# NJU-RLC/quadrupedal-agility

Hardware: AMD Instinct MI355X
Metric: env-steps/sec (4096 Go2 envs) + wall-clock to 1k PPO iters, 1/2/4/8 GPU (higher is better)
Workload: dtype f32

## Files before the change

### __graft_entry__.py

```python
import os
import shutil
import subprocess
import sys

ROOT = os.path.dirname(os.path.abspath(__file__))
CSRC = os.path.join(ROOT, "quadrupedal_agility_amd", "csrc")
if ROOT not in sys.path:
    sys.path.insert(0, ROOT)


def _hipcc():
    for cand in (shutil.which("hipcc"), "/opt/rocm/bin/hipcc"):
        if cand and os.path.exists(cand):
            return cand
    raise RuntimeError("hipcc not found")


def _src_hash(srcs):
    import hashlib
    h = hashlib.sha256()
    for s in srcs:
        h.update(os.path.basename(s).encode()); h.update(open(s, "rb").read())
    return h.hexdigest()


def _stale(out, srcs):
    stamp = out + ".srchash"
    if not os.path.exists(out) or not os.path.exists(stamp):
        return True
    return open(stamp).read().strip() != _src_hash(srcs)


HIP_SOURCES = (("qa_sim.hip", ["-fno-slp-vectorize", "-fno-hip-fp32-correctly-rounded-divide-sqrt"]), ("qa_learner.hip", []), ("qa_gemm.hip", []), ("qa_conv.hip", []),
               ("qa_policy.hip", []), ("qa_tsc.hip", ["-ffp-contract=off"]), ("qa_depth.hip", []))
HIP_HEADERS = ("qa_physics.h", "qa_device.h", "qa_go2_model.h", "qa_rewards.h")


def _lib_sources():
    srcs = [os.path.join(CSRC, f) for f, _ in HIP_SOURCES] + [os.path.join(CSRC, f) for f in HIP_HEADERS]
    srcs.append(os.path.join(ROOT, "include", "qa_sim.h"))
    srcs.append(os.path.join(ROOT, "include", "qa_sim_curriculum.h"))
    srcs.append(os.path.join(ROOT, "include", "qa_tsc_curriculum.h"))
    srcs.append(os.path.join(ROOT, "include", "qa_sim_rewards.h"))
    return srcs


def compile_library(out, obj_dir=None):
    base = [_hipcc(), "--offload-arch=gfx950", "-O3", "-std=c++17", "-fPIC"]
    obj_dir = obj_dir or os.path.dirname(out)
    objs = []
    for src, extra in HIP_SOURCES:
        obj = os.path.join(obj_dir, src.replace(".hip", ".o"))
        subprocess.check_call(base + extra + ["-c", os.path.join(CSRC, src), "-o", obj])
        objs.append(obj)
    subprocess.check_call([_hipcc(), "--offload-arch=gfx950", "-shared", "-fPIC", "-o", out] + objs)
    for obj in objs:
        os.remove(obj)


def build():
    srcs = _lib_sources()
    out = os.path.join(CSRC, "libqa_sim.so")
    if os.environ.get("QA_FORCE_REBUILD") == "1" or _stale(out, srcs):
        compile_library(out)
        with open(out + ".srchash", "w") as f:
            f.write(_src_hash(srcs))
    subprocess.check_call(["make", "-C", os.path.join(ROOT, "oracle"), "-s"])
    import quadrupedal_agility_amd
    from quadrupedal_agility_amd import _capi
    lib = _capi.load_library()
    assert lib.qa_abi_version() == _capi.QA_ABI_VERSION


def smoke():
    import numpy as np
    import torch
    from tests.oracle_lib import OracleSim, go2_cfg
    from quadrupedal_agility_amd.sim import QaSim
    assert torch.cuda.is_available(), "smoke() needs a GPU"
    n = 64
    q = go2_cfg(n, seed=1)
    o = OracleSim(q)
    h = QaSim(q, "cuda:0")
    o.reset_all()
    rng = np.random.default_rng(0)
    for _ in range(3):
        h.arena.copy_(torch.from_numpy(o.arena.copy()).cuda()); h.global_step = o.global_step
        act = rng.normal(0, 1, (n, 12)).astype(np.float32)
        o.step(act); h.step(torch.from_numpy(act).cuda())
        torch.cuda.synchronize()
        from tests.parity_tol import MEDIAN_TOL, env_mismatch, env_errors
        bad = np.zeros(n, bool)
        for name in ("OBS", "REW", "ROOT_STATES", "DOF_STATE", "OBS_DISC"):
            got, exp = h.t[name].cpu().numpy(), o.t[name]
            bad |= env_mismatch(name, got, exp, n)
            med = float(np.median(env_errors(name, got, exp, n)))
# ... 64 lines not shown
```

### quadrupedal_agility_amd/_capi.py

```python
import ctypes as C
import os

import torch

QA_ABI_VERSION = 18
NUM_DOF = 12
NUM_GAITS = 5
NUM_PROP = 57
HISTORY_LEN = 10
NUM_OBS = 671
NUM_OBS_DISC = 49
ACTION_BUF_LEN = 8
NUM_REWARDS = 14
MOCAP_FRAME = 37
MAX_MOCAP_CLIPS, MOCAP_CLIP = 64, 8
OBST_SEESAW, OBST_BAR, OBST_TYRE = 1, 2, 3

REWARD_NAMES = [
    "action_rate", "collision", "delta_torques", "dof_acc", "dof_error", "dof_pos_limits",
    "dof_vel_limits", "hip_pos", "jump_up_height", "locomotion_height", "torque_limits",
    "torques", "tracking_ang_vel", "tracking_lin_vel",
]

EXTRA_REWARD_NAMES = [
# ... 160 lines not shown
    f = getattr(lib, prefix + "tsc_goal_step"); f.argtypes = [C.c_void_p, C.c_void_p, C.c_void_p]; f.restype = C.c_int
    f = getattr(lib, prefix + "tsc_observations"); f.argtypes = [C.c_void_p, C.c_void_p, C.c_void_p]; f.restype = C.c_int
    f = getattr(lib, prefix + "tsc_depth_update"); f.argtypes = [C.c_void_p, C.c_void_p, C.c_void_p]; f.restype = C.c_int
    f = getattr(lib, prefix + "mlp_packed_floats"); f.argtypes = [C.c_void_p, C.c_int32]; f.restype = C.c_int64
    f = getattr(lib, prefix + "mlp_pack"); f.argtypes = [C.c_void_p, C.c_int32, C.c_void_p, C.c_void_p, C.c_void_p, C.c_int64, C.c_void_p]; f.restype = C.c_int
    f = getattr(lib, prefix + "mlp_strands"); f.argtypes = [C.c_void_p, C.c_int32, C.c_int32, C.c_void_p]; f.restype = C.c_int
    f = getattr(lib, prefix + "mlp_groups"); f.argtypes = [C.c_void_p, C.c_int32, C.c_int32, C.c_void_p, C.c_void_p, C.c_void_p, C.c_void_p]; f.restype = C.c_int
    f = getattr(lib, prefix + "mlp_set_groups"); f.argtypes = [C.c_int32]; f.restype = C.c_int
    f = getattr(lib, prefix + "mlp_forward")
    f.argtypes = [C.c_void_p, C.c_int64, C.c_int32, C.c_int32, C.c_void_p, C.c_int32, C.c_void_p, C.c_void_p, C.c_void_p, C.c_int32, C.c_void_p]
    f.restype = C.c_int
    f = getattr(lib, prefix + "elu_backward_bias")
    f.argtypes = [C.c_void_p] * 4 + [C.c_int64, C.c_int32, C.c_float, C.c_void_p, C.c_int64, C.c_void_p]
    f.restype = C.c_int
    f = getattr(lib, prefix + "narrow_wgrad_scratch_bytes"); f.argtypes = [C.c_int64, C.c_int32, C.c_int32]; f.restype = C.c_int64
    f = getattr(lib, prefix + "linear_forward")
    f.argtypes = [C.c_void_p, C.c_int64, C.c_void_p, C.c_int64, C.c_void_p, C.c_void_p, C.c_int64, C.c_int64, C.c_int32, C.c_int32, C.c_int32, C.c_float, C.c_void_p]
    f.restype = C.c_int
    f = getattr(lib, prefix + "linear_backward_input")
    f.argtypes = [C.c_void_p, C.c_int64, C.c_void_p, C.c_int64, C.c_void_p, C.c_int64, C.c_void_p, C.c_int64, C.c_int64, C.c_int32, C.c_int32, C.c_int32, C.c_float, C.c_void_p]
    f.restype = C.c_int
    f = getattr(lib, prefix + "linear_backward_weight_scratch_bytes"); f.argtypes = [C.c_int64, C.c_int32, C.c_int32]; f.restype = C.c_int64
    f = getattr(lib, prefix + "linear_backward_weight_layout"); f.argtypes = [C.c_int64, C.c_int32, C.c_int32, C.c_void_p]; f.restype = C.c_int
    f = getattr(lib, prefix + "linear_backward_weight_batch_layout"); f.argtypes = [C.c_int64, C.c_int32, C.c_int32, C.c_void_p]; f.restype = C.c_int
    f = getattr(lib, prefix + "linear_backward_weight_batch_scratch_bytes"); f.argtypes = [C.c_int64, C.c_int32, C.c_int32]; f.restype = C.c_int64
    f = getattr(lib, prefix + "linear_backward_weight_batch"); f.argtypes = [C.c_void_p, C.c_int32, C.c_void_p]; f.restype = C.c_int
    f = getattr(lib, prefix + "linear_backward_weight")
    f.argtypes = [C.c_void_p, C.c_int64, C.c_void_p, C.c_int64, C.c_void_p, C.c_void_p, C.c_int64, C.c_int32, C.c_int32, C.c_void_p, C.c_int64, C.c_void_p]
    f.restype = C.c_int
    f = getattr(lib, prefix + "tsc_reset_stats"); f.argtypes = [C.c_void_p, C.c_void_p, C.c_int64, C.c_int32, C.c_float, C.c_void_p, C.c_void_p, C.c_void_p]; f.restype = C.c_int
    f = getattr(lib, prefix + "slab_sum"); f.argtypes = [C.c_void_p, C.c_int64, C.c_int32, C.c_int64, C.c_void_p, C.c_void_p]; f.restype = C.c_int
    P, I64, I32, FL = C.c_void_p, C.c_int64, C.c_int32, C.c_float
    f = getattr(lib, prefix + "linear_forward_split_scratch_bytes"); f.argtypes = [I64, I32, I32]; f.restype = C.c_int64
    f = getattr(lib, prefix + "linear_forward_split"); f.argtypes = [P, I64, P, I64, P, P, I64, I64, I32, I32, I32, FL, P, I64, P]; f.restype = C.c_int
    f = getattr(lib, prefix + "disc_sample_prepare"); f.argtypes = [C.POINTER(QaDiscSampleIo), I32, I32, P, P, P, P, P, FL, FL, P, P]; f.restype = C.c_int
    f = getattr(lib, prefix + "disc_step_tail_scratch_bytes"); f.argtypes = []; f.restype = C.c_int64
    f = getattr(lib, prefix + "disc_step_tail"); f.argtypes = [P, P, I64, I32, P, P, I32, P, P, P, P, I32, FL, P, I64, P]; f.restype = C.c_int
    f = getattr(lib, prefix + "depth_stem_forward"); f.argtypes = [P, P, P, P, P, I64, I32, I32, FL, P]; f.restype = C.c_int
    f = getattr(lib, prefix + "depth_stem_backward_scratch_bytes"); f.argtypes = []; f.restype = C.c_int64
    f = getattr(lib, prefix + "depth_stem_backward"); f.argtypes = [P, P, P, P, I64, I32, I32, P, I64, P]; f.restype = C.c_int
    f = getattr(lib, prefix + "conv_nhwc_forward"); f.argtypes = [P, P, P, P, I64, I32, I32, I32, I32, I32, I32, I32, FL, P]; f.restype = C.c_int
    f = getattr(lib, prefix + "conv_nhwc_backward_input"); f.argtypes = [P, P, P, P, I64, I32, I32, I32, I32, I32, I32, I32, FL, P]; f.restype = C.c_int
    f = getattr(lib, prefix + "conv_nhwc_backward_weight_scratch_bytes"); f.argtypes = [I64, I32, I32, I32, I32, I32, I32]; f.restype = C.c_int64
    f = getattr(lib, prefix + "conv_nhwc_backward_weight"); f.argtypes = [P, P, P, P, I64, I32, I32, I32, I32, I32, I32, P, I64, P]; f.restype = C.c_int
    f = getattr(lib, prefix + "elu_backward_pad"); f.argtypes = [P, P, P, P, I64, I32, I32, I32, I32, I32, FL, P]; f.restype = C.c_int
    f = getattr(lib, prefix + "narrow_wgrad"); f.argtypes = [C.c_void_p, C.c_void_p, C.c_int64, C.c_int32, C.c_int32, C.c_void_p, C.c_void_p, C.c_void_p, C.c_int64, C.c_void_p]; f.restype = C.c_int
    return lib


def bind_extensions(lib, prefix="qa_"):
    f = getattr(lib, prefix + "set_terrain_curriculum"); f.argtypes = [C.c_void_p] * 4 + [C.c_int32, C.c_int32, C.c_float, C.c_float]; f.restype = C.c_int
    f = getattr(lib, prefix + "tsc_obstacle_curriculum"); f.argtypes = [C.POINTER(QaTscObstCurr), C.c_void_p]; f.restype = C.c_int
    f = getattr(lib, prefix + "set_extra_rewards"); f.argtypes = [C.c_void_p, C.POINTER(QaExtraRewards)]; f.restype = C.c_int
    return lib


class QaExtraRewards(C.Structure):
    _fields_ = [("scale_dt", C.c_float * 10), ("base_height_target", C.c_float), ("max_contact_force", C.c_float), ("step_dt", C.c_float),
                ("num_scan_points", C.c_int32), ("scan_offsets", C.c_void_p), ("extra_episode_sums", C.c_void_p), ("feet_air_time", C.c_void_p),
                ("extra_episode_stats", C.c_void_p)]


class QaTscObstCurr(C.Structure):
    _fields_ = [("step_counter", C.c_void_p), ("counter_offset", C.c_void_p), ("success_rate", C.c_void_p), ("any_reset", C.c_void_p),
                ("threshold", C.c_double), ("period", C.c_int64), ("state", C.c_void_p), ("ticket", C.c_void_p), ("increments", C.c_void_p),
                ("biases", C.c_void_p), ("last", C.c_int32), ("reserved", C.c_int32),
                ("cell_index", C.c_void_p), ("cell_kind", C.c_void_p), ("cell_base", C.c_void_p), ("num_cells", C.c_int64),
                ("height_samples", C.c_void_p), ("scan_samples", C.c_void_p), ("map_cells", C.c_int64),
                ("ceiling_index", C.c_void_p), ("ceiling_base", C.c_void_p), ("num_ceiling_cells", C.c_int64), ("ceiling_samples", C.c_void_p),
                ("goal_index", C.c_void_p), ("goal_kind", C.c_void_p), ("goal_base", C.c_void_p), ("num_goal_entries", C.c_int64),
                ("env_goals", C.c_void_p), ("goal_floats", C.c_int64)]


TSC_OBST_BAR, TSC_OBST_TYRE, TSC_OBST_STATE_WORDS = 0, 1, 4


class QaMlpOp(C.Structure):
    _fields_ = [("kind", C.c_int32), ("src_buf", C.c_int32), ("src_col", C.c_int32), ("dst_buf", C.c_int32), ("dst_col", C.c_int32),
                ("k", C.c_int32), ("n", C.c_int32), ("act", C.c_int32), ("out_index", C.c_int32), ("flags", C.c_int32),
                ("w_off", C.c_int64), ("b_off", C.c_int64), ("out_col", C.c_int32), ("aux_index", C.c_int32), ("aux_col", C.c_int32), ("pad_", C.c_int32)]


class QaWgradDesc(C.Structure):
    _fields_ = [("grad_out", C.c_void_p), ("ldg", C.c_int64), ("x", C.c_void_p), ("ldx", C.c_int64), ("grad_weight", C.c_void_p), ("grad_bias", C.c_void_p),
                ("rows", C.c_int64), ("in_features", C.c_int32), ("out_features", C.c_int32), ("scratch", C.c_void_p), ("scratch_bytes", C.c_int64)]


ADAM_STACK_MAX_TENSORS, ADAM_STACK_MAX_STATES = 16, 3


class QaPairJob(C.Structure):
    _fields_ = [("a", C.c_void_p), ("b", C.c_void_p), ("rows", C.c_int64), ("cols", C.c_int32), ("mode", C.c_int32), ("b_stride", C.c_int64),
                ("grad_scale", C.c_void_p), ("grad_a", C.c_void_p), ("out", C.c_void_p)]


class QaAdamPair(C.Structure):
    _fields_ = [("split_tensor", C.c_int32), ("split_chunk", C.c_int32), ("lr2", C.c_void_p), ("max_norm2", C.c_float), ("kl", C.c_void_p),
                ("desired_kl", C.c_float), ("kl_factor", C.c_float), ("lr_min", C.c_float), ("lr_max", C.c_float)]


class QaAdamStackState(C.Structure):
    _fields_ = [("exp_avg", C.c_void_p), ("exp_avg_sq", C.c_void_p), ("step", C.c_void_p), ("lr", C.c_void_p), ("weight_decay", C.c_float), ("pad_", C.c_int32)]


class QaAdamStackTensor(C.Structure):
    _fields_ = [("param", C.c_void_p), ("grad", C.c_void_p), ("tmp", C.c_void_p), ("src1", C.c_void_p), ("src2", C.c_void_p), ("stride1", C.c_int64), ("stride2", C.c_int64),
                ("parts1", C.c_int32), ("parts2", C.c_int32), ("alpha2", C.c_float), ("reg", C.c_float), ("numel", C.c_int32), ("num_states", C.c_int32),
# ... 24 lines not shown


TSC_GOAL_IO_FIELDS = ("root_states", "contact_forces", "rigid_body_states", "env_goals", "obstacle_types", "action_hl_history", "x_edge_mask",
                      "episode_length", "cur_goal_idx", "reach_goal_timer", "last_contacts", "cur_goals", "next_goals", "episode_sums",
                      "base_lin_vel", "base_ang_vel", "projected_gravity", "rpy", "contact_filt", "target_pos_rel", "next_target_pos_rel",
                      "target_yaw", "next_target_yaw", "reached_goal", "cur_obstacle_type", "reset_buf", "time_out_buf", "reach_goal_cutoff",
                      "rew_buf")


class QaTscGoalIo(C.Structure):
    _fields_ = [(name, C.c_void_p) for name in TSC_GOAL_IO_FIELDS]


class QaTscObsCfg(C.Structure):
    _fields_ = [("num_envs", C.c_int64), ("num_bodies", C.c_int32), ("key_bodies", C.c_int32 * 4), ("map_rows", C.c_int32), ("map_cols", C.c_int32),
                ("update_yaw", C.c_int32), ("root_height_obs", C.c_int32), ("action_stride", C.c_int64),
                ("points_env_stride", C.c_int64), ("point_stride", C.c_int32), ("reserved", C.c_int32),
                ("border_size", C.c_float), ("horizontal_scale", C.c_float), ("vertical_scale", C.c_float),
                ("lin_vel", C.c_float), ("ang_vel", C.c_float), ("dof_pos", C.c_float), ("dof_vel", C.c_float), ("lin_vel_dist", C.c_float),
                ("ang_vel_dist", C.c_float), ("key_pos", C.c_float), ("foot_contact", C.c_float), ("clip_observations", C.c_float),
                ("default_dof_pos", C.c_float * 12), ("default_dof_pos_all", C.c_float * 12)]


TSC_OBS_IO_FIELDS = ("root_states", "rpy", "base_lin_vel", "base_ang_vel", "contact_filt", "dof_pos", "dof_vel", "last_action",
                     "rigid_body_states", "mass_params", "friction", "motor_strength", "cur_obstacle_type", "target_yaw", "next_target_yaw",
                     "height_samples", "height_points", "commands", "latent_eps", "latent_c", "episode_length", "delta_yaw", "delta_next_yaw",
                     "obs_history", "measured_heights", "obs_buf", "obs_bbc_buf", "obs_disc_buf")
TSC_NUM_SCAN, TSC_NUM_OBS, TSC_NUM_OBS_BBC, TSC_NUM_OBS_DISC = 132, 800, 671, 49


class QaTscObsIo(C.Structure):
    _fields_ = [(name, C.c_void_p) for name in TSC_OBS_IO_FIELDS]


class QaTscDepthCfg(C.Structure):
    _fields_ = [("num_envs", C.c_int64), ("step", C.c_int64), ("seed", C.c_uint64), ("env_id_offset", C.c_int32), ("width", C.c_int32),
                ("height", C.c_int32), ("crop_top", C.c_int32), ("crop_bottom", C.c_int32), ("crop_left", C.c_int32), ("crop_right", C.c_int32),
                ("buffer_len", C.c_int32), ("map_rows", C.c_int32), ("map_cols", C.c_int32), ("coarse_log2", C.c_int32),
                ("horizontal_fov_deg", C.c_float), ("position", C.c_float * 3), ("near_clip", C.c_float), ("far_clip", C.c_float),
                ("depth_noise", C.c_float), ("border_size", C.c_float), ("horizontal_scale", C.c_float), ("vertical_scale", C.c_float)]


TSC_DEPTH_IO_FIELDS = ("root_states", "camera_pitch", "height_samples", "ceiling_samples", "episode_length", "depth_buffer", "coarse_floor_max",
                       "coarse_ceiling_min", "step_dev")


class QaTscDepthIo(C.Structure):
    _fields_ = [(name, C.c_void_p) for name in TSC_DEPTH_IO_FIELDS]


ABI_SYMBOLS = ["arena_bytes", "create", "destroy", "tensor_info", "env_step", "env_step_dev", "reset_all", "simulate",
               "set_mocap", "debug_post_physics", "env_physics_step", "tsc_reset", "tsc_reset_dev", "simulate_if", "gae", "ppo_loss", "ppo_loss_scratch_bytes", "hybrid_ppo_loss", "hybrid_ppo_loss_scratch_bytes", "elu_backward_bias",
               "elu_backward_bias_scratch_bytes", "narrow_wgrad", "narrow_wgrad_scratch_bytes", "linear_forward", "linear_backward_input", "linear_backward_weight", "linear_backward_weight_scratch_bytes", "linear_backward_weight_layout", "linear_backward_weight_batch", "linear_backward_weight_batch_layout", "linear_backward_weight_batch_scratch_bytes", "slab_sum", "linear_forward_split", "linear_forward_split_scratch_bytes", "depth_stem_forward", "depth_stem_backward", "depth_stem_backward_scratch_bytes", "conv_nhwc_forward", "conv_nhwc_backward_input", "conv_nhwc_backward_weight", "conv_nhwc_backward_weight_scratch_bytes", "elu_backward_pad", "normalizer_update", "normalizer_apply", "clip_adam_step", "clip_adam_step_hostgrads", "clip_adam_step_reduce", "clip_adam_pair_step", "grad_reduce", "adam_stack_step", "rollout_act", "rollout_act_store", "rollout_act_hybrid", "rollout_post", "rollout_post_amp", "disc_loss", "disc_loss_logits", "disc_loss_scratch_bytes", "disc_prepare", "disc_sample_prepare", "disc_step_tail", "disc_step_tail_scratch_bytes", "pair_loss", "pair_loss_scratch_bytes", "pair_losses", "pair_losses_scratch_bytes", "accumulate_scalars", "gather_rows", "kl_lr_rule", "episode_means", "set_lean_exports", "mlp_packed_floats", "mlp_pack", "mlp_forward", "mlp_strands", "mlp_groups", "mlp_set_groups", "tsc_set_commands", "tsc_goal_step", "tsc_observations", "tsc_depth_update", "tsc_reset_stats", "tsc_push", "tsc_start_pose", "tsc_reset_where", "last_error", "abi_version"]
EXTENSION_SYMBOLS = ["set_terrain_curriculum", "tsc_obstacle_curriculum", "set_extra_rewards"]

_LIB = None
LIB_PATH = os.environ.get("QA_LIB") or os.path.join(os.path.dirname(os.path.abspath(__file__)), "csrc", "libqa_sim.so")


def load_library():
    global _LIB
    if _LIB is None:
        if not os.path.exists(LIB_PATH):
            raise RuntimeError(
                f"{LIB_PATH} is missing: build it with `python -c 'import __graft_entry__ as g; g.build()'` "
                "(hipcc --offload-arch=gfx950). quadrupedal_agility_amd has no CPU fallback.")
        lib = C.CDLL(LIB_PATH)
        bind(lib, "qa_")
        bind_extensions(lib, "qa_")
        lib.qa_last_error.restype = C.c_char_p
        lib.qa_abi_version.restype = C.c_int
        if lib.qa_abi_version() != QA_ABI_VERSION:
            raise RuntimeError("libqa_sim.so ABI version mismatch")
        _LIB = lib
    return _LIB


def tensor_info(lib, prefix, cfg, which):
    off = C.c_int64(); shape = (C.c_int64 * 3)(); nd = C.c_int32(); dt = C.c_int32()
    rc = getattr(lib, prefix + "tensor_info")(C.byref(cfg), which, C.byref(off), shape, C.byref(nd), C.byref(dt))
    if rc != 0:
        raise RuntimeError(f"{prefix}tensor_info({which}) -> {rc}")
    return off.value, tuple(shape[i] for i in range(nd.value)), dt.value


def _ptr(t):
    return C.c_void_p(t.data_ptr())


def stream(on):
    dev = on if type(on) is torch.device else on.device
    return C.c_void_p(torch.cuda.current_stream(dev).cuda_stream) if dev.type == "cuda" else None


NO_ERROR_TEXT = "(an injected library: no error text)"


class Api:

    stream = staticmethod(stream)

    def __init__(self, lib=None, prefix="qa_"):
        self._lib, self.prefix = lib, prefix
        self._fns = {}

    @property
    def lib(self):
# ... 41 lines not shown
```

### quadrupedal_agility_amd/csrc/qa_learner.hip

```cpp
#include <hip/hip_runtime.h>
#include <stdint.h>
#include <stdio.h>

#include "../../include/qa_sim.h"
#include "../../include/qa_tsc_curriculum.h"
#include "qa_device.h"

namespace {

constexpr int PPO_BLOCK = 64;
constexpr int PPO_D = 12;
constexpr int PPO_SUMS = 5 + PPO_D;

struct PpoArgs {
    const float *mu, *std, *value, *actions, *old_logp, *old_mu, *old_sigma, *adv, *returns, *target_values;
    float *dmu, *dvalue;
    float *partial;
    int64_t B;
    float clip, c_surr, c_value, c_bound, c_entropy;
    int clipped_value;
};

__device__ __forceinline__ float wave_sum(float v) {
#pragma unroll
    for (int o = 32; o > 0; o >>= 1) v += __shfl_xor(v, o, 64);
    return v;
}

__global__ void __launch_bounds__(PPO_BLOCK) qa_ppo_loss_kernel(PpoArgs a) {
    const int64_t i = (int64_t)blockIdx.x * PPO_BLOCK + threadIdx.x;
    const bool live = i < a.B;
    const int64_t r = live ? i : a.B - 1;
    const float invB = 1.0f / (float)a.B;
    float sd[PPO_D];
#pragma unroll
    for (int j = 0; j < PPO_D; ++j) sd[j] = a.std[j];
    float mu[PPO_D], ac[PPO_D], omu[PPO_D], osd[PPO_D];
    {
        const float4 *m4 = (const float4 *)(a.mu + r * PPO_D), *a4 = (const float4 *)(a.actions + r * PPO_D);
        const float4 *om4 = (const float4 *)(a.old_mu + r * PPO_D), *os4 = (const float4 *)(a.old_sigma + r * PPO_D);
#pragma unroll
        for (int q = 0; q < 3; ++q) {
            float4 m = m4[q], x = a4[q], om = om4[q], os = os4[q];
            mu[4 * q] = m.x; mu[4 * q + 1] = m.y; mu[4 * q + 2] = m.z; mu[4 * q + 3] = m.w;
            ac[4 * q] = x.x; ac[4 * q + 1] = x.y; ac[4 * q + 2] = x.z; ac[4 * q + 3] = x.w;
            omu[4 * q] = om.x; omu[4 * q + 1] = om.y; omu[4 * q + 2] = om.z; omu[4 * q + 3] = om.w;
            osd[4 * q] = os.x; osd[4 * q + 1] = os.y; osd[4 * q + 2] = os.z; osd[4 * q + 3] = os.w;
        }
    }
    const float v = a.value[r], adv = a.adv[r], ret = a.returns[r], tv = a.target_values[r], ologp = a.old_logp[r];

    const float HALF_LOG_2PI = 0.91893853320467274178f;
    float logp = 0.f, ent = 0.f, kl = 0.f, bl = 0.f;
    float dlogp_dmu[PPO_D], dlogp_dsd[PPO_D], dbl_dmu[PPO_D];
#pragma unroll
    for (int j = 0; j < PPO_D; ++j) {
        const float s = sd[j], inv_s = 1.0f / s, d = ac[j] - mu[j], var = s * s, ls = logf(s);
        logp += -(d * d) / (2.0f * var) - ls - HALF_LOG_2PI;
        ent += 0.5f + HALF_LOG_2PI + ls;
        const float dm = omu[j] - mu[j];
        kl += logf(s / osd[j] + 1.0e-5f) + (osd[j] * osd[j] + dm * dm) / (2.0f * var) - 0.5f;
        dlogp_dmu[j] = d / var;
        dlogp_dsd[j] = d * d * inv_s * inv_s * inv_s - inv_s;
        const float lo = fminf(mu[j] + 1.0f, 0.0f), hi = fmaxf(mu[j] - 1.0f, 0.0f);
        bl += lo * lo + hi * hi;
        dbl_dmu[j] = 2.0f * lo + 2.0f * hi;
    }
    const float ratio = expf(logp - ologp);
    const float rc = fminf(fmaxf(ratio, 1.0f - a.clip), 1.0f + a.clip);
    const float s1 = -adv * ratio, s2 = -adv * rc;
    const float surr = fmaxf(s1, s2);
    const bool inside = ratio >= 1.0f - a.clip && ratio <= 1.0f + a.clip;
    float dsurr_dratio = s1 > s2 ? -adv : (s1 == s2 ? (inside ? -adv : -0.5f * adv) : 0.0f);
    const float dsurr_dlogp = dsurr_dratio * ratio;
    float vl, dvl_dv;
    if (a.clipped_value) {
        const float dv = v - tv, dvc = fminf(fmaxf(dv, -a.clip), a.clip), vc = tv + dvc;
        const float l1 = (v - ret) * (v - ret), l2 = (vc - ret) * (vc - ret);
        const float pass = (dv >= -a.clip && dv <= a.clip) ? 1.0f : 0.0f;
        vl = fmaxf(l1, l2);
        dvl_dv = l1 > l2 ? 2.0f * (v - ret) : (l1 == l2 ? (v - ret) + (vc - ret) * pass : 2.0f * (vc - ret) * pass);
    } else {
        vl = (ret - v) * (ret - v);
        dvl_dv = 2.0f * (v - ret);
    }
    if (live) {
        float g[PPO_D];
#pragma unroll
        for (int j = 0; j < PPO_D; ++j) g[j] = invB * (a.c_surr * dsurr_dlogp * dlogp_dmu[j] + a.c_bound * dbl_dmu[j]);
        float4 *o4 = (float4 *)(a.dmu + r * PPO_D);
        o4[0] = make_float4(g[0], g[1], g[2], g[3]); o4[1] = make_float4(g[4], g[5], g[6], g[7]); o4[2] = make_float4(g[8], g[9], g[10], g[11]);
        a.dvalue[r] = invB * a.c_value * dvl_dv;
    }
    const float w = live ? 1.0f : 0.0f;
    float part[PPO_SUMS];
    part[0] = w * surr; part[1] = w * vl; part[2] = w * bl; part[3] = w * ent; part[4] = w * kl;
#pragma unroll
    for (int j = 0; j < PPO_D; ++j) part[5 + j] = w * (a.c_surr * dsurr_dlogp * dlogp_dsd[j] - a.c_entropy / sd[j]);
#pragma unroll
    for (int k = 0; k < PPO_SUMS; ++k) {
        float s = wave_sum(part[k]);
        if (threadIdx.x == k) a.partial[(int64_t)blockIdx.x * PPO_SUMS + k] = s;
    }
}

__global__ void __launch_bounds__(256) qa_ppo_finish_kernel(const float *partial, int nblocks, int64_t B, float c_surr, float c_value,
                                                            float c_bound, float c_entropy, float *out, float *dstd) {
    constexpr int LANES = 256 / PPO_SUMS;
    __shared__ double s_acc[256];
    __shared__ double s_tot[PPO_SUMS];
    const int t = threadIdx.x;
    const int k = t / LANES, l = t % LANES;
    double acc = 0.0;
    if (k < PPO_SUMS)
        for (int b = l; b < nblocks; b += LANES) acc += (double)partial[(int64_t)b * PPO_SUMS + k];
    s_acc[t] = acc;
    __syncthreads();
    if (k < PPO_SUMS && l == 0) {
        double tot = 0.0;
        for (int q = 0; q < LANES; ++q) tot += s_acc[k * LANES + q];
        s_tot[k] = tot;
    }
    __syncthreads();
    const double invB = 1.0 / (double)B;
    if (t < 5) out[1 + t] = (float)(s_tot[t] * invB);
    if (t == 5) out[0] = (float)((c_surr * s_tot[0] + c_value * s_tot[1] + c_bound * s_tot[2] - c_entropy * s_tot[3]) * invB);
    if (t == 6 || t == 7) out[t] = 0.f;
    if (t >= 8 && t < 8 + PPO_D) dstd[t - 8] = (float)(s_tot[5 + t - 8] * invB);
}

constexpr int HYB_ND = 3, HYB_NC = 18, HYB_SUMS = 5 + HYB_NC;
struct HybArgs {
    const float *logits, *mean, *std, *value, *actions, *old_logp_d, *old_logp_c, *old_mu, *old_sigma, *adv, *returns, *target_values;
    float *dlogits, *dmean, *dvalue, *partial;
    int64_t B;
    float clip, c_value, c_entropy;
    int clipped_value;
};
__device__ __forceinline__ void clipped_surrogate(float logp, float ologp, float adv, float clip, float &surr, float &dsurr_dlogp) {
    const float ratio = expf(logp - ologp), rc = fminf(fmaxf(ratio, 1.0f - clip), 1.0f + clip);
    const float s1 = -adv * ratio, s2 = -adv * rc;
    surr = fmaxf(s1, s2);
    const bool inside = ratio >= 1.0f - clip && ratio <= 1.0f + clip;
    const float d = s1 > s2 ? -adv : (s1 == s2 ? (inside ? -adv : -0.5f * adv) : 0.0f);
    dsurr_dlogp = d * ratio;
}
__global__ void __launch_bounds__(PPO_BLOCK) qa_hybrid_ppo_loss_kernel(HybArgs a) {
    const int64_t i = (int64_t)blockIdx.x * PPO_BLOCK + threadIdx.x;
    const bool live = i < a.B;
    const int64_t r = live ? i : a.B - 1;
    const float invB = 1.0f / (float)a.B;
    const float HALF_LOG_2PI = 0.91893853320467274178f, EPS = 1.1920928955078125e-07f;
    float z[HYB_ND], pr[HYB_ND], lp[HYB_ND], fl[HYB_ND];
    float zmax = -3.0e38f;
#pragma unroll
    for (int k = 0; k < HYB_ND; ++k) { z[k] = a.logits[r * HYB_ND + k]; zmax = fmaxf(zmax, z[k]); }
    float den = 0.f;
#pragma unroll
    for (int k = 0; k < HYB_ND; ++k) { pr[k] = expf(z[k] - zmax); den += pr[k]; }
    float Hd = 0.f, sum_pf = 0.f;
#pragma unroll
    for (int k = 0; k < HYB_ND; ++k) {
        pr[k] /= den;
        fl[k] = (pr[k] > EPS && pr[k] < 1.0f - EPS) ? 1.0f : 0.0f;
        lp[k] = logf(fminf(fmaxf(pr[k], EPS), 1.0f - EPS));
        Hd -= pr[k] * lp[k];
        sum_pf += pr[k] * fl[k];
    }
    const float *act = a.actions + r * (1 + HYB_NC);
    int ad = (int)act[0];
    ad = ad < 0 ? 0 : (ad >= HYB_ND ? HYB_ND - 1 : ad);
    const float lpa = ad == 0 ? lp[0] : (ad == 1 ? lp[1] : lp[2]);
    const float fa = ad == 0 ? fl[0] : (ad == 1 ? fl[1] : fl[2]);
    const float adv = a.adv[r];
    float surr_d, dsd_dlogp;
    clipped_surrogate(lpa, a.old_logp_d[r], adv, a.clip, surr_d, dsd_dlogp);
    float logp = 0.f, ent_c = 0.f, kl = 0.f;
    float dlogp_dmu[HYB_NC], dlogp_dsd[HYB_NC], inv_sd[HYB_NC];
#pragma unroll
    for (int j = 0; j < HYB_NC; ++j) {
        const float s = a.std[j], inv_s = 1.0f / s, mu = a.mean[r * HYB_NC + j], d = act[1 + j] - mu, var = s * s, ls = logf(s);
// ... 295 lines not shown
    int num_chunks, num_tensors;
    float beta1, beta2, eps, max_norm;
    int inline_grads;
    const float *gin[QA_ADAM_MAX_INLINE];
    int has_reduce;
    const float *red_src[QA_ADAM_MAX_INLINE];
    int64_t red_stride[QA_ADAM_MAX_INLINE];
    int32_t red_parts[QA_ADAM_MAX_INLINE];
    int split_chunk, split_tensor;
    float *lr2; float max_norm2;
    const float *kl; float desired_kl, kl_factor, lr_min, lr_max;
};
__device__ __forceinline__ const float *adam_grad(const AdamArgs &a, int t) { return a.inline_grads ? a.gin[t] : a.grads[t]; }

constexpr int QA_REDUCE_WIDE = 16;
__device__ __forceinline__ float adam_reduce_chunk(const float *__restrict__ src, int64_t stride, int parts, float *__restrict__ g, int n, float *s_q) {
    float acc = 0.f;
    if (parts <= QA_REDUCE_WIDE) {
        for (int i = threadIdx.x; i < n; i += 256) {
            float v[QA_REDUCE_WIDE];
#pragma unroll
            for (int z = 0; z < QA_REDUCE_WIDE; ++z) v[z] = z < parts ? src[(int64_t)z * stride + i] : 0.f;
            float s = v[0];
#pragma unroll
            for (int z = 1; z < QA_REDUCE_WIDE; ++z) if (z < parts) s += v[z];
            g[i] = s;
            acc = fmaf(s, s, acc);
        }
    } else {
        const int c = threadIdx.x & 31, q = threadIdx.x >> 5;
        float a0 = 0.f, a1 = 0.f, a2 = 0.f, a3 = 0.f;
        if (c < n) {
            int b = q;
            for (; b + 24 < parts; b += 32) {
                a0 += src[(int64_t)b * stride + c]; a1 += src[(int64_t)(b + 8) * stride + c];
                a2 += src[(int64_t)(b + 16) * stride + c]; a3 += src[(int64_t)(b + 24) * stride + c];
            }
            for (; b < parts; b += 8) a0 += src[(int64_t)b * stride + c];
        }
        s_q[threadIdx.x] = (a0 + a1) + (a2 + a3);
        __syncthreads();
        if (q == 0 && c < n) {
            float t = 0.f;
#pragma unroll
            for (int k = 0; k < 8; ++k) t += s_q[threadIdx.x + 32 * k];
            g[c] = t;
            acc = t * t;
        }
        __syncthreads();
    }
    return acc;
}

__global__ void __launch_bounds__(256) qa_adam_sumsq_kernel(AdamArgs a) {
    __shared__ float s_w[4];
    __shared__ float s_q[256];
    const int c = blockIdx.x, t = a.chunk_tensor[c];
    const float *g = adam_grad(a, t) + a.chunk_start[c];
    const int n = a.chunk_len[c];
    float acc = 0.f;
    if (a.has_reduce && a.red_parts[t] > 0) {
        acc = adam_reduce_chunk(a.red_src[t] + a.chunk_start[c], a.red_stride[t], a.red_parts[t], const_cast<float *>(g), n, s_q);
    } else {
        for (int i = threadIdx.x; i < n; i += 256) { const float v = g[i]; acc = fmaf(v, v, acc); }
    }
    acc = wave_sum(acc);
    if ((threadIdx.x & 63) == 0) s_w[threadIdx.x >> 6] = acc;
    __syncthreads();
    if (threadIdx.x == 0) a.scratch[4 + c] = (s_w[0] + s_w[1]) + (s_w[2] + s_w[3]);
}

__global__ void __launch_bounds__(256) qa_adam_finalize_kernel(AdamArgs a) {
    __shared__ double s_acc[256], s_acc2[256];
    const int split = a.split_chunk > 0 ? a.split_chunk : a.num_chunks;
    double acc = 0.0, acc2 = 0.0;
    if (a.max_norm > 0.f)
        for (int c = threadIdx.x; c < split; c += 256) acc += (double)a.scratch[4 + c];
    if (a.split_chunk > 0 && a.max_norm2 > 0.f)
        for (int c = split + threadIdx.x; c < a.num_chunks; c += 256) acc2 += (double)a.scratch[4 + c];
    s_acc[threadIdx.x] = acc; s_acc2[threadIdx.x] = acc2;
    __syncthreads();
    for (int o = 128; o > 0; o >>= 1) { if (threadIdx.x < o) { s_acc[threadIdx.x] += s_acc[threadIdx.x + o]; s_acc2[threadIdx.x] += s_acc2[threadIdx.x + o]; } __syncthreads(); }
    const int nt1 = a.split_chunk > 0 ? a.split_tensor : a.num_tensors;
    const float step = a.steps[0][0] + 1.0f;
    const float step2 = a.split_chunk > 0 ? a.steps[nt1][0] + 1.0f : 0.f;
    __syncthreads();
    for (int t = threadIdx.x; t < a.num_tensors; t += 256) a.steps[t][0] = t < nt1 ? step : step2;
    if (threadIdx.x == 0) {
        const float norm = (float)sqrt(s_acc[0]);
        a.scratch[0] = a.max_norm > 0.f ? fminf(1.0f, a.max_norm / (norm + 1e-6f)) : 1.0f;
        a.scratch[1] = 1.0f - powf(a.beta1, step);
        a.scratch[2] = sqrtf(1.0f - powf(a.beta2, step));
        a.scratch[3] = norm;
        if (a.split_chunk > 0) {
            float *h = a.scratch + 4 + a.num_chunks + 1;
            const float norm2 = (float)sqrt(s_acc2[0]);
            h[0] = a.max_norm2 > 0.f ? fminf(1.0f, a.max_norm2 / (norm2 + 1e-6f)) : 1.0f;
            h[1] = 1.0f - powf(a.beta1, step2);
            h[2] = sqrtf(1.0f - powf(a.beta2, step2));
            h[3] = norm2;
            if (a.kl) {
                const float k = a.kl[0], cur = a.lr2[0];
                float out = cur;
                if (k > a.desired_kl * 2.0f) out = fmaxf(a.lr_min, cur / a.kl_factor);
                else if (k < a.desired_kl / 2.0f && k > 0.0f) out = fminf(a.lr_max, cur * a.kl_factor);
                a.lr2[0] = out;
            }
        }
    }
}

constexpr int PAIR_BLOCK = 256;

__global__ void __launch_bounds__(PAIR_BLOCK) qa_pair_loss_kernel(const float *__restrict__ a, const float *__restrict__ b, int64_t rows, int cols,
                                                                 int64_t b_stride, int mode, float *__restrict__ grad_a, float *__restrict__ partial) {
    __shared__ float s_red[PAIR_BLOCK];
    const int64_t r = (int64_t)blockIdx.x * PAIR_BLOCK + threadIdx.x;
    float contrib = 0.f;
    if (r < rows) {
        const float *ar = a + r * cols, *br = b + r * b_stride;
        float *gr = grad_a + r * cols;
        float ss = 0.f;
        for (int c = 0; c < cols; ++c) { const float d = ar[c] - br[c]; ss = fmaf(d, d, ss); }
        if (mode == 0) {
            const float nrm = sqrtf(ss);
            const float sc = nrm > 0.f ? 1.0f / (nrm * (float)rows) : 0.f;
            for (int c = 0; c < cols; ++c) gr[c] = (ar[c] - br[c]) * sc;
            contrib = nrm;
        } else {
            const float sc = 2.0f / ((float)rows * (float)cols);
            for (int c = 0; c < cols; ++c) gr[c] = (ar[c] - br[c]) * sc;
            contrib = ss;
        }
    }
    s_red[threadIdx.x] = contrib;
    __syncthreads();
    for (int o = PAIR_BLOCK / 2; o > 0; o >>= 1) { if (threadIdx.x < o) s_red[threadIdx.x] += s_red[threadIdx.x + o]; __syncthreads(); }
    if (threadIdx.x == 0) partial[blockIdx.x] = s_red[0];
}

__global__ void __launch_bounds__(256) qa_pair_finish_kernel(const float *__restrict__ partial, int nb, float scale, float *__restrict__ out) {
    __shared__ double s_acc[256];
    double acc = 0.0;
    for (int i = threadIdx.x; i < nb; i += 256) acc += (double)partial[i];
    s_acc[threadIdx.x] = acc;
    __syncthreads();
    for (int o = 128; o > 0; o >>= 1) { if (threadIdx.x < o) s_acc[threadIdx.x] += s_acc[threadIdx.x + o]; __syncthreads(); }
    if (threadIdx.x == 0) out[0] = (float)(s_acc[0] * (double)scale);
}

constexpr int PAIR_LDS_COLS = 47;
struct PairJobsArgs { qa_pair_job j[QA_PAIR_MAX_JOBS]; int32_t first_block[QA_PAIR_MAX_JOBS + 1]; int32_t n; float *partial; unsigned *ticket; };
__global__ void __launch_bounds__(PAIR_BLOCK) qa_pair_losses_kernel(PairJobsArgs p) {
    __shared__ float s_red[PAIR_BLOCK];
    __shared__ double s_acc[PAIR_BLOCK];
    __shared__ int s_last;
    __shared__ float s_d[PAIR_BLOCK * (PAIR_LDS_COLS | 1)];
    int t = 0;
    while (t + 1 < p.n && (int)blockIdx.x >= p.first_block[t + 1]) ++t;
    const float *a = p.j[t].a, *b = p.j[t].b;
    const int64_t rows = p.j[t].rows, b_stride = p.j[t].b_stride;
    const int cols = p.j[t].cols, mode = p.j[t].mode;
    const bool scaled = p.j[t].grad_scale != nullptr;
// ... 51 lines not shown
    if (threadIdx.x == 0) {
        p.partial[blockIdx.x] = s_red[0];
        __threadfence();
        s_last = atomicAdd(p.ticket, 1u) == (unsigned)(p.first_block[p.n] - 1);
    }
    __syncthreads();
    if (!s_last) return;
    __threadfence();
    for (int k = 0; k < p.n; ++k) {
        const int lo = p.first_block[k], nb = p.first_block[k + 1] - lo;
        double acc = 0.0;
        for (int i = threadIdx.x; i < nb; i += 256) acc += (double)__hip_atomic_load(p.partial + lo + i, __ATOMIC_RELAXED, __HIP_MEMORY_SCOPE_AGENT);
        s_acc[threadIdx.x] = acc;
        __syncthreads();
        for (int o = 128; o > 0; o >>= 1) { if (threadIdx.x < o) s_acc[threadIdx.x] += s_acc[threadIdx.x + o]; __syncthreads(); }
        if (threadIdx.x == 0) {
            const float scale = p.j[k].mode == QA_PAIR_ROW_L2 ? 1.0f / (float)p.j[k].rows : 1.0f / ((float)p.j[k].rows * (float)p.j[k].cols);
            p.j[k].out[0] = (float)(s_acc[0] * (double)scale);
        }
        __syncthreads();
    }
    if (threadIdx.x == 0) *p.ticket = 0u;
}

constexpr int GATHER_ROWS = 4;
struct GatherArgs {
    const float *src[QA_GATHER_MAX]; float *dst[QA_GATHER_MAX]; int32_t width[QA_GATHER_MAX]; int64_t src_stride[QA_GATHER_MAX];
    const int64_t *idx; const int64_t *idx_block; int64_t rows; int32_t n;
};

__global__ void __launch_bounds__(256) qa_gather_rows_kernel(GatherArgs a) {
    const int lane = threadIdx.x & 63;
    const int64_t r = (int64_t)blockIdx.x * GATHER_ROWS + (threadIdx.x >> 6);
    if (r >= a.rows) return;
    const int64_t s = a.idx[(a.idx_block ? a.idx_block[0] * a.rows : 0) + r];
    for (int t = 0; t < a.n; ++t) {
        const float *sp = a.src[t] + s * a.src_stride[t];
        float *dp = a.dst[t] + r * a.width[t];
        const int w = a.width[t];
        if (w <= 64) { if (lane < w) dp[lane] = sp[lane]; continue; }
        int c = lane;
        for (; c + 192 < w; c += 256) {
            const float v0 = sp[c], v1 = sp[c + 64], v2 = sp[c + 128], v3 = sp[c + 192];
            dp[c] = v0; dp[c + 64] = v1; dp[c + 128] = v2; dp[c + 192] = v3;
        }
        for (; c < w; c += 64) dp[c] = sp[c];
    }
}

struct AccArgs { float *acc; const float *src[QA_ACC_MAX]; int n; };
__global__ void qa_accumulate_scalars_kernel(AccArgs a) {
    const int i = threadIdx.x;
    if (i < a.n) a.acc[i] += a.src[i][0];
}

__global__ void qa_kl_lr_rule_kernel(const float *kl, float desired_kl, float factor, float lr_min, float lr_max, float *lr) {
    const float k = kl[0], cur = lr[0];
    float out = cur;
    if (k > desired_kl * 2.0f) out = fmaxf(lr_min, cur / factor);
    else if (k < desired_kl / 2.0f && k > 0.0f) out = fminf(lr_max, cur * factor);
    lr[0] = out;
}

__global__ void qa_episode_means_kernel(const float *__restrict__ stats, const int64_t *__restrict__ step_dev, int64_t step, int num_terms,
                                        float max_len_s, float *__restrict__ means, float *__restrict__ snapshot) {
    const int i = threadIdx.x;
    if (i >= num_terms) return;
    const int64_t st = step_dev ? step_dev[0] : step;
    const float *b = stats + 16 * (int)((st - 1) & 1);
    const float cnt = b[14];
    const float m = cnt > 0.f ? b[i] / fmaxf(cnt, 1.0f) / max_len_s : means[i];
    means[i] = m;
    snapshot[i] = m;
}

template <bool SELF>
__global__ void __launch_bounds__(256) qa_adam_update_kernel(AdamArgs a) {
    const int c = blockIdx.x, t = a.chunk_tensor[c], s0 = a.chunk_start[c], n = a.chunk_len[c];
    float *p = a.params[t] + s0, *m = a.exp_avg[t] + s0, *v = a.exp_avg_sq[t] + s0;
    const float *g = adam_grad(a, t) + s0;
    const float step = SELF ? a.steps[0][0] + 1.0f : 0.f;
    const bool second = !SELF && a.split_chunk > 0 && c >= a.split_chunk;
    const float *head = second ? a.scratch + 4 + a.num_chunks + 1 : a.scratch;
    const float coef = SELF ? 1.0f : head[0], bc1 = SELF ? 1.0f - powf(a.beta1, step) : head[1],
                bc2s = SELF ? sqrtf(1.0f - powf(a.beta2, step)) : head[2], wd = a.weight_decay[t];
    const float step_size = (second ? a.lr2[0] : a.lr[0]) / bc1;
    for (int i = threadIdx.x; i < n; i += 256) {
        const float pi = p[i];
        const float gi = fmaf(wd, pi, g[i] * coef);
        const float mi = a.beta1 * m[i] + (1.0f - a.beta1) * gi;
        const float vi = a.beta2 * v[i] + (1.0f - a.beta2) * gi * gi;
        m[i] = mi; v[i] = vi;
        p[i] = pi - step_size * mi / (sqrtf(vi) / bc2s + a.eps);
    }
    if (SELF) {
        __syncthreads();
        if (threadIdx.x == 0) {
            unsigned *ticket = (unsigned *)(a.scratch + 4 + a.num_chunks);
            __threadfence();
            if (atomicAdd(ticket, 1u) == (unsigned)(a.num_chunks - 1)) {
                for (int k = 0; k < a.num_tensors; ++k) a.steps[k][0] = step;
                a.scratch[0] = 1.0f; a.scratch[1] = bc1; a.scratch[2] = bc2s; a.scratch[3] = 0.f;
                *ticket = 0u;
            }
        }
    }
// ... 517 lines not shown
    if (i >= total) return;
    const int64_t r = i / a.dim; const int c = (int)(i - r * a.dim);
    const float *src; int64_t rr = r;
    if (rr < a.rows[0]) src = a.src[0];
    else if ((rr -= a.rows[0]) < a.rows[1]) src = a.src[1];
    else { rr -= a.rows[1]; src = a.src[2]; }
    float x = src[rr * a.dim + c];
    if (a.task_w && a.task_mask[c] != 0.f) x *= a.task_w[0];
    x *= a.frame_mult[c];
    if (a.mean) {
        const float m = (float)a.mean[c], sd = sqrtf((float)(a.var[c] + (double)a.eps));
        x = fminf(fmaxf((x - m) / sd, -a.clip), a.clip);
    }
    a.out[i] = x;
}

struct SampleArgs {
    qa_disc_sample_io io;
    int dim, c_dim;
    const float *task_mask, *frame_mult, *task_w; const double *mean, *var; float eps, clip; float *out;
    int64_t main_blocks;
};

__global__ void __launch_bounds__(256) qa_disc_sample_prepare_kernel(SampleArgs a) {
    const qa_disc_sample_io &io = a.io;
    const int64_t blk = io.block_dev[0];
    if ((int64_t)blockIdx.x < a.main_blocks) {
        const int64_t total = (io.rows[0] + io.rows[1] + io.rows[2]) * a.dim;
        const int64_t i = (int64_t)blockIdx.x * 256 + threadIdx.x;
        if (i >= total) return;
        const int64_t r = i / a.dim; const int c = (int)(i - r * a.dim);
        int b = 0; int64_t rr = r;
        if (rr >= io.rows[0]) { rr -= io.rows[0]; b = 1; if (rr >= io.rows[1]) { rr -= io.rows[1]; b = 2; } }
        const int64_t row = io.index[b][blk * io.rows[b] + rr];
        float x = io.src[b][row * a.dim + c];
        if (a.task_w && a.task_mask[c] != 0.f) x *= a.task_w[0];
        x *= a.frame_mult[c];
        if (a.mean) {
            const float m = (float)a.mean[c], sd = sqrtf((float)(a.var[c] + (double)a.eps));
            x = fminf(fmaxf((x - m) / sd, -a.clip), a.clip);
        }
        a.out[i] = x;
        return;
    }
    const int64_t j = ((int64_t)blockIdx.x - a.main_blocks) * 256 + threadIdx.x;
    if (j < io.rows[1] && io.eps_src) {
        const int64_t row = io.index[1][blk * io.rows[1] + j];
        io.eps_out[j] = io.eps_src[row];
        for (int k = 0; k < a.c_dim; ++k) io.c_out[j * a.c_dim + k] = io.c_src[row * a.c_dim + k];
    }
    if (j < io.rows[0] && io.label_src) io.label_out[j] = io.label_src[blk * io.rows[0] + j];
}

}

extern thread_local char qa_err_buf[512];
#define g_lerr qa_err_buf

extern "C" {

int64_t qa_ppo_loss_scratch_bytes(int64_t B) { return B <= 0 ? -1 : (int64_t)sizeof(float) * PPO_SUMS * ((B + PPO_BLOCK - 1) / PPO_BLOCK); }

int qa_ppo_loss(const float *mu, const float *std, const float *value, const float *actions, const float *old_logp,
                const float *old_mu, const float *old_sigma, const float *advantages, const float *returns,
                const float *target_values, int64_t B, int32_t num_actions, float clip, float c_surr, float c_value,
                float c_bound, float c_entropy, int32_t clipped_value, float *dmu, float *dstd, float *dvalue, float *out,
                void *scratch, int64_t scratch_bytes, void *stream) {
    if (!mu || !std || !value || !actions || !old_logp || !old_mu || !old_sigma || !advantages || !returns || !target_values ||
        !dmu || !dstd || !dvalue || !out || !scratch || B <= 0) { snprintf(g_lerr, sizeof(g_lerr), "qa_ppo_loss: null pointer or empty batch"); return QA_E_ARG; }
    if (num_actions != PPO_D) { snprintf(g_lerr, sizeof(g_lerr), "qa_ppo_loss: num_actions must be %d", PPO_D); return QA_E_ARG; }
    if ((((uintptr_t)mu | (uintptr_t)actions | (uintptr_t)old_mu | (uintptr_t)old_sigma | (uintptr_t)dmu) & 15) != 0) {
        snprintf(g_lerr, sizeof(g_lerr), "qa_ppo_loss: (B,12) tensors must be 16-byte aligned"); return QA_E_ARG; }
    hipStream_t st = (hipStream_t)stream;
    const int blocks = (int)((B + PPO_BLOCK - 1) / PPO_BLOCK);
    if (scratch_bytes < qa_ppo_loss_scratch_bytes(B)) { snprintf(g_lerr, sizeof(g_lerr), "qa_ppo_loss: scratch too small"); return QA_E_ARG; }
    PpoArgs a{mu, std, value, actions, old_logp, old_mu, old_sigma, advantages, returns, target_values, dmu, dvalue, (float *)scratch,
              B, clip, c_surr, c_value, c_bound, c_entropy, clipped_value};
    hipLaunchKernelGGL(qa_ppo_loss_kernel, dim3(blocks), dim3(PPO_BLOCK), 0, st, a);
    hipLaunchKernelGGL(qa_ppo_finish_kernel, dim3(1), dim3(256), 0, st, (const float *)scratch, blocks, B, c_surr, c_value, c_bound, c_entropy, out, dstd);
    hipError_t e = hipGetLastError();
    if (e != hipSuccess) { snprintf(g_lerr, sizeof(g_lerr), "qa_ppo_loss: %s", hipGetErrorString(e)); return QA_E_DEVICE; }
    return QA_OK;
}

int64_t qa_hybrid_ppo_loss_scratch_bytes(int64_t B) { return B <= 0 ? -1 : (int64_t)sizeof(float) * HYB_SUMS * ((B + PPO_BLOCK - 1) / PPO_BLOCK); }

int qa_hybrid_ppo_loss(const float *logits, const float *mean, const float *std, const float *value, const float *actions, const float *old_logp_d,
                       const float *old_logp_c, const float *old_mu, const float *old_sigma, const float *advantages, const float *returns,
                       const float *target_values, int64_t B, int32_t num_d, int32_t num_c, float clip, float c_value, float c_entropy,
                       int32_t clipped_value, float *dlogits, float *dmean, float *dstd, float *dvalue, float *out, void *scratch,
                       int64_t scratch_bytes, void *stream) {
    if (!logits || !mean || !std || !value || !actions || !old_logp_d || !old_logp_c || !old_mu || !old_sigma || !advantages || !returns ||
        !target_values || !dlogits || !dmean || !dstd || !dvalue || !out || !scratch || B <= 0) {
        snprintf(g_lerr, sizeof(g_lerr), "qa_hybrid_ppo_loss: null pointer or empty batch"); return QA_E_ARG; }
    if (num_d != HYB_ND || num_c != HYB_NC) { snprintf(g_lerr, sizeof(g_lerr), "qa_hybrid_ppo_loss: built for num_d = %d, num_c = %d", HYB_ND, HYB_NC); return QA_E_ARG; }
    if (scratch_bytes < qa_hybrid_ppo_loss_scratch_bytes(B)) { snprintf(g_lerr, sizeof(g_lerr), "qa_hybrid_ppo_loss: scratch too small"); return QA_E_ARG; }
    hipStream_t st = (hipStream_t)stream;
    const int blocks = (int)((B + PPO_BLOCK - 1) / PPO_BLOCK);
    HybArgs a{logits, mean, std, value, actions, old_logp_d, old_logp_c, old_mu, old_sigma, advantages, returns, target_values, dlogits, dmean, dvalue,
              (float *)scratch, B, clip, c_value, c_entropy, clipped_value};
    hipLaunchKernelGGL(qa_hybrid_ppo_loss_kernel, dim3(blocks), dim3(PPO_BLOCK), 0, st, a);
    hipLaunchKernelGGL(qa_hybrid_ppo_finish_kernel, dim3(1), dim3(256), 0, st, (const float *)scratch, blocks, B, c_value, c_entropy, out, dstd);
    hipError_t e = hipGetLastError();
    if (e != hipSuccess) { snprintf(g_lerr, sizeof(g_lerr), "qa_hybrid_ppo_loss: %s", hipGetErrorString(e)); return QA_E_DEVICE; }
    return QA_OK;
}

int64_t qa_elu_backward_bias_scratch_bytes(int64_t rows, int32_t cols) {
    return (rows <= 0 || cols <= 0) ? -1 : (int64_t)sizeof(float) * cols * ((rows + ELU_ROWS - 1) / ELU_ROWS);
}

int qa_elu_backward_bias(const float *grad_out, const float *out, float *grad_in, float *grad_bias, int64_t rows, int32_t cols,
                         float alpha, void *scratch, int64_t scratch_bytes, void *stream) {
    if (!grad_out || !out || !grad_in || !scratch || rows <= 0 || cols <= 0) { snprintf(g_lerr, sizeof(g_lerr), "qa_elu_backward_bias: bad argument"); return QA_E_ARG; }
    if (scratch_bytes < qa_elu_backward_bias_scratch_bytes(rows, cols)) { snprintf(g_lerr, sizeof(g_lerr), "qa_elu_backward_bias: scratch too small"); return QA_E_ARG; }
    hipStream_t st = (hipStream_t)stream;
    const int nb = (int)((rows + ELU_ROWS - 1) / ELU_ROWS);
    float *partial = (float *)scratch;
    if (cols > 128) hipLaunchKernelGGL(qa_elu_bwd_bias_kernel<256>, dim3(nb), dim3(256), 0, st, grad_out, out, grad_in, partial, rows, (int)cols, alpha);
    else if (cols > 64) hipLaunchKernelGGL(qa_elu_bwd_bias_kernel<128>, dim3(nb), dim3(256), 0, st, grad_out, out, grad_in, partial, rows, (int)cols, alpha);
    else if (cols > 32) hipLaunchKernelGGL(qa_elu_bwd_bias_kernel<64>, dim3(nb), dim3(256), 0, st, grad_out, out, grad_in, partial, rows, (int)cols, alpha);
    else hipLaunchKernelGGL(qa_elu_bwd_bias_kernel<32>, dim3(nb), dim3(256), 0, st, grad_out, out, grad_in, partial, rows, (int)cols, alpha);
    if (grad_bias) hipLaunchKernelGGL(qa_colsum_finish_kernel, dim3((cols + 31) / 32), dim3(256), 0, st, (const float *)partial, nb, (int)cols, grad_bias);
    hipError_t e = hipGetLastError();
    if (e != hipSuccess) { snprintf(g_lerr, sizeof(g_lerr), "qa_elu_backward_bias: %s", hipGetErrorString(e)); return QA_E_DEVICE; }
    return QA_OK;
}

static int narrow_slabs(int64_t rows, int *slab_rows) {
    int sr = (int)((rows + 255) / 256);
    sr = sr < 8 ? 8 : (sr > NARROW_MAX_SLAB ? NARROW_MAX_SLAB : sr);
    *slab_rows = sr;
    return (int)((rows + sr - 1) / sr);
}
// ... 1 lines not shown
    int sr; const int nb = narrow_slabs(rows, &sr);
    return (int64_t)nb * ((int64_t)out_features * in_features + out_features) * 4;
}
int qa_narrow_wgrad(const float *grad_out, const float *x, int64_t rows, int32_t O, int32_t K, float *grad_weight, float *grad_bias,
                    void *scratch, int64_t scratch_bytes, void *stream) {
    if (!grad_out || !x || !grad_weight || !grad_bias || !scratch || rows <= 0 || O <= 0 || O > QA_NARROW_MAX_OUT || K <= 0) {
        snprintf(g_lerr, sizeof(g_lerr), "qa_narrow_wgrad: bad argument (1 <= out_features <= %d)", QA_NARROW_MAX_OUT); return QA_E_ARG; }
    if (scratch_bytes < qa_narrow_wgrad_scratch_bytes(rows, O, K)) { snprintf(g_lerr, sizeof(g_lerr), "qa_narrow_wgrad: scratch too small"); return QA_E_ARG; }
    hipStream_t st = (hipStream_t)stream;
    int sr; const int nb = narrow_slabs(rows, &sr);
    float *partial = (float *)scratch;
    if (O <= 1) hipLaunchKernelGGL(qa_narrow_wgrad_kernel<1>, dim3(nb), dim3(256), 0, st, grad_out, x, rows, sr, (int)O, (int)K, partial);
    else if (O <= 4) hipLaunchKernelGGL(qa_narrow_wgrad_kernel<4>, dim3(nb), dim3(256), 0, st, grad_out, x, rows, sr, (int)O, (int)K, partial);
    else if (O <= 16) hipLaunchKernelGGL(qa_narrow_wgrad_kernel<16>, dim3(nb), dim3(256), 0, st, grad_out, x, rows, sr, (int)O, (int)K, partial);
    else hipLaunchKernelGGL(qa_narrow_wgrad_kernel<32>, dim3(nb), dim3(256), 0, st, grad_out, x, rows, sr, (int)O, (int)K, partial);
    const int cols = O * K + O;
    hipLaunchKernelGGL(qa_colsum_finish2_kernel, dim3((cols + 31) / 32), dim3(256), 0, st, (const float *)partial, nb, cols, O * K, grad_weight, grad_bias);
    hipError_t e = hipGetLastError();
    if (e != hipSuccess) { snprintf(g_lerr, sizeof(g_lerr), "qa_narrow_wgrad: %s", hipGetErrorString(e)); return QA_E_DEVICE; }
    return QA_OK;
}

int qa_normalizer_update(const float *const *batches, const int64_t *rows, int32_t num_batches, int32_t dim,
                         double *mean, double *var, double *count, void *stream) {
    if (!batches || !rows || !mean || !var || !count || num_batches <= 0 || num_batches > NORM_MAX_BATCHES || dim <= 0 || dim > 128) {
        snprintf(g_lerr, sizeof(g_lerr), "qa_normalizer_update: bad argument (1..4 batches, dim <= 128)"); return QA_E_ARG; }
    NormArgs a{};
    for (int b = 0; b < num_batches; ++b) {
        if (!batches[b] || rows[b] <= 0) { snprintf(g_lerr, sizeof(g_lerr), "qa_normalizer_update: empty batch"); return QA_E_ARG; }
        a.batch[b] = batches[b]; a.n[b] = rows[b];
    }
    a.k = num_batches; a.d = dim; a.mean = mean; a.var = var; a.count = count;
    hipLaunchKernelGGL(qa_normalizer_update_kernel, dim3((dim + 15) / 16), dim3(1024), 0, (hipStream_t)stream, a);
    hipLaunchKernelGGL(qa_normalizer_count_kernel, dim3(1), dim3(1), 0, (hipStream_t)stream, a);
    hipError_t e = hipGetLastError();
    if (e != hipSuccess) { snprintf(g_lerr, sizeof(g_lerr), "qa_normalizer_update: %s", hipGetErrorString(e)); return QA_E_DEVICE; }
    return QA_OK;
}

int qa_normalizer_apply(const float *x, float *y, int64_t rows, int32_t dim, const double *mean, const double *var,
                        float epsilon, float clip, void *stream) {
    if (!x || !y || !mean || !var || rows <= 0 || dim <= 0) { snprintf(g_lerr, sizeof(g_lerr), "qa_normalizer_apply: bad argument"); return QA_E_ARG; }
    const int64_t total = rows * dim;
    hipLaunchKernelGGL(qa_normalizer_apply_kernel, dim3((unsigned)((total + 255) / 256)), dim3(256), 0, (hipStream_t)stream, x, y, total, (int)dim, mean, var, epsilon, clip);
    hipError_t e = hipGetLastError();
    if (e != hipSuccess) { snprintf(g_lerr, sizeof(g_lerr), "qa_normalizer_apply: %s", hipGetErrorString(e)); return QA_E_DEVICE; }
    return QA_OK;
}

static int clip_adam_launch(float *const *params, const float *const *grads_dev, const float *const *grads_host, float *const *exp_avg,
                            float *const *exp_avg_sq, float *const *steps, int32_t num_tensors, const int32_t *chunk_tensor, const int32_t *chunk_start,
                            const int32_t *chunk_len, int32_t num_chunks, const float *weight_decay, const float *lr, float beta1, float beta2, float eps,
                            float max_norm, float *scratch, int64_t scratch_floats, void *stream, const char *who,
                            const float *const *red_src = nullptr, const int64_t *red_stride = nullptr, const int32_t *red_parts = nullptr, const qa_adam_pair *pair = nullptr) {
    if (!params || (!grads_dev && !grads_host) || !exp_avg || !exp_avg_sq || !steps || !chunk_tensor || !chunk_start || !chunk_len || !weight_decay || !lr ||
        !scratch || num_tensors <= 0 || num_chunks <= 0 || scratch_floats < 4 + (int64_t)num_chunks || (grads_host && num_tensors > QA_ADAM_MAX_INLINE)) {
        snprintf(g_lerr, sizeof(g_lerr), "%s: bad argument", who); return QA_E_ARG; }
    AdamArgs a{};
    a.params = params; a.grads = grads_dev; a.exp_avg = exp_avg; a.exp_avg_sq = exp_avg_sq; a.steps = steps; a.chunk_tensor = chunk_tensor; a.chunk_start = chunk_start;
    a.chunk_len = chunk_len; a.weight_decay = weight_decay; a.lr = lr; a.scratch = scratch; a.num_chunks = num_chunks; a.num_tensors = num_tensors;
    a.beta1 = beta1; a.beta2 = beta2; a.eps = eps; a.max_norm = max_norm; a.inline_grads = grads_host ? 1 : 0;
    if (pair) {
        if (!grads_host || pair->split_tensor <= 0 || pair->split_tensor >= num_tensors || pair->split_chunk <= 0 || pair->split_chunk >= num_chunks || !pair->lr2 ||
            !(max_norm > 0.f) || !(pair->max_norm2 > 0.f) || scratch_floats < 4 + (int64_t)num_chunks + 1 + 4) {
            snprintf(g_lerr, sizeof(g_lerr), "%s: two clipping optimisers (max_norm > 0 both), the host pointer form, 0 < split < count and scratch >= num_chunks + 9 floats expected", who);
            return QA_E_ARG; }
        a.split_chunk = pair->split_chunk; a.split_tensor = pair->split_tensor; a.lr2 = pair->lr2; a.max_norm2 = pair->max_norm2;
        a.kl = pair->kl; a.desired_kl = pair->desired_kl; a.kl_factor = pair->kl_factor; a.lr_min = pair->lr_min; a.lr_max = pair->lr_max;
    }
    if (grads_host) for (int t = 0; t < num_tensors; ++t) a.gin[t] = grads_host[t];
    if (red_src) {
        if (!grads_host || !(max_norm > 0.f) || !red_parts || !red_stride) {
            snprintf(g_lerr, sizeof(g_lerr), "%s: gradients in parts need the host pointer form and a clipping step (max_norm > 0): the parts are added by the sums-of-squares pass", who);
            return QA_E_ARG; }
        for (int t = 0; t < num_tensors; ++t) {
            if (red_parts[t] < 0 || (red_parts[t] > 0 && (!red_src[t] || red_stride[t] <= 0))) { snprintf(g_lerr, sizeof(g_lerr), "%s: bad parts record of tensor %d", who, t); return QA_E_ARG; }
            a.red_src[t] = red_src[t]; a.red_stride[t] = red_stride[t]; a.red_parts[t] = red_parts[t];
            if (red_parts[t] > 0) a.has_reduce = 1;
        }
    }
    hipStream_t st = (hipStream_t)stream;
    if (!(max_norm > 0.f) && scratch_floats >= 5 + (int64_t)num_chunks) {
        hipLaunchKernelGGL(qa_adam_update_kernel<true>, dim3(num_chunks), dim3(256), 0, st, a);
    } else {
        if (max_norm > 0.f) hipLaunchKernelGGL(qa_adam_sumsq_kernel, dim3(num_chunks), dim3(256), 0, st, a);
        hipLaunchKernelGGL(qa_adam_finalize_kernel, dim3(1), dim3(256), 0, st, a);
        hipLaunchKernelGGL(qa_adam_update_kernel<false>, dim3(num_chunks), dim3(256), 0, st, a);
    }
    hipError_t e = hipGetLastError();
    if (e != hipSuccess) { snprintf(g_lerr, sizeof(g_lerr), "%s: %s", who, hipGetErrorString(e)); return QA_E_DEVICE; }
    return QA_OK;
}

int qa_clip_adam_step(float *const *params, const float *const *grads, float *const *exp_avg, float *const *exp_avg_sq,
                      float *const *steps, int32_t num_tensors, const int32_t *chunk_tensor, const int32_t *chunk_start,
                      const int32_t *chunk_len, int32_t num_chunks, const float *weight_decay, const float *lr, float beta1,
                      float beta2, float eps, float max_norm, float *scratch, int64_t scratch_floats, void *stream) {
    return clip_adam_launch(params, grads, nullptr, exp_avg, exp_avg_sq, steps, num_tensors, chunk_tensor, chunk_start, chunk_len, num_chunks, weight_decay, lr,
                            beta1, beta2, eps, max_norm, scratch, scratch_floats, stream, "qa_clip_adam_step");
}

int qa_clip_adam_step_hostgrads(float *const *params, const float *const *grads_host, float *const *exp_avg, float *const *exp_avg_sq,
                                float *const *steps, int32_t num_tensors, const int32_t *chunk_tensor, const int32_t *chunk_start,
                                const int32_t *chunk_len, int32_t num_chunks, const float *weight_decay, const float *lr, float beta1,
                                float beta2, float eps, float max_norm, float *scratch, int64_t scratch_floats, void *stream) {
    return clip_adam_launch(params, nullptr, grads_host, exp_avg, exp_avg_sq, steps, num_tensors, chunk_tensor, chunk_start, chunk_len, num_chunks, weight_decay,
                            lr, beta1, beta2, eps, max_norm, scratch, scratch_floats, stream, "qa_clip_adam_step_hostgrads");
}

int qa_clip_adam_step_reduce(float *const *params, const float *const *grads_host, float *const *exp_avg, float *const *exp_avg_sq,
                             float *const *steps, int32_t num_tensors, const int32_t *chunk_tensor, const int32_t *chunk_start,
                             const int32_t *chunk_len, int32_t num_chunks, const float *weight_decay, const float *lr, float beta1,
                             float beta2, float eps, float max_norm, float *scratch, int64_t scratch_floats,
                             const float *const *red_src_host, const int64_t *red_stride_host, const int32_t *red_parts_host, void *stream) {
    if (!red_src_host || !red_stride_host || !red_parts_host) { snprintf(g_lerr, sizeof(g_lerr), "qa_clip_adam_step_reduce: bad argument"); return QA_E_ARG; }
    return clip_adam_launch(params, nullptr, grads_host, exp_avg, exp_avg_sq, steps, num_tensors, chunk_tensor, chunk_start, chunk_len, num_chunks, weight_decay,
                            lr, beta1, beta2, eps, max_norm, scratch, scratch_floats, stream, "qa_clip_adam_step_reduce", red_src_host, red_stride_host, red_parts_host);
}

int qa_clip_adam_pair_step(float *const *params, const float *const *grads_host, float *const *exp_avg, float *const *exp_avg_sq,
                           float *const *steps, int32_t num_tensors, const int32_t *chunk_tensor, const int32_t *chunk_start,
                           const int32_t *chunk_len, int32_t num_chunks, const float *weight_decay, const float *lr, float beta1,
                           float beta2, float eps, float max_norm, float *scratch, int64_t scratch_floats,
                           const float *const *red_src_host, const int64_t *red_stride_host, const int32_t *red_parts_host, const qa_adam_pair *pair, void *stream) {
    if (!pair) { snprintf(g_lerr, sizeof(g_lerr), "qa_clip_adam_pair_step: bad argument"); return QA_E_ARG; }
    return clip_adam_launch(params, nullptr, grads_host, exp_avg, exp_avg_sq, steps, num_tensors, chunk_tensor, chunk_start, chunk_len, num_chunks, weight_decay,
                            lr, beta1, beta2, eps, max_norm, scratch, scratch_floats, stream, "qa_clip_adam_pair_step", red_src_host, red_stride_host, red_parts_host, pair);
}

struct ReduceArgs { float *dst[QA_ADAM_MAX_INLINE]; const float *src[QA_ADAM_MAX_INLINE]; int64_t stride[QA_ADAM_MAX_INLINE]; int32_t parts[QA_ADAM_MAX_INLINE];
                    int32_t numel[QA_ADAM_MAX_INLINE]; int32_t first_block[QA_ADAM_MAX_INLINE + 1]; int32_t n; };
__global__ void __launch_bounds__(256) qa_grad_reduce_kernel(ReduceArgs a) {
    __shared__ float s_q[256];
    int t = 0;
    while (t + 1 < a.n && (int)blockIdx.x >= a.first_block[t + 1]) ++t;
// ... 362 lines not shown
    small = io->rows[0] > io->rows[1] ? io->rows[0] : io->rows[1];
    SampleArgs a{};
    a.io = *io; a.dim = dim; a.c_dim = c_dim; a.task_mask = task_mask; a.frame_mult = frame_mult; a.task_w = task_weight_dev; a.mean = mean; a.var = var;
    a.eps = epsilon; a.clip = clip; a.out = out; a.main_blocks = (total + 255) / 256;
    const int64_t extra = (io->eps_src || io->label_src) ? (small + 255) / 256 : 0;
    hipLaunchKernelGGL(qa_disc_sample_prepare_kernel, dim3((unsigned)(a.main_blocks + extra)), dim3(256), 0, (hipStream_t)stream, a);
    hipError_t e = hipGetLastError();
    if (e != hipSuccess) { snprintf(g_lerr, sizeof(g_lerr), "qa_disc_sample_prepare: %s", hipGetErrorString(e)); return QA_E_DEVICE; }
    return QA_OK;
}

int64_t qa_disc_step_tail_scratch_bytes(void) { return (int64_t)(TAIL_MAX * TAIL_WG + 4) * 4; }

int qa_disc_step_tail(const float *head_stats, const float *input_grad, int64_t grad_rows, int32_t grad_cols, const float *const *weights,
                      const int64_t *weight_counts, int32_t num_weights, float *out, float *acc, int64_t *step_counter, float *prior, int32_t prior_dim,
                      float prior_soft_coef, void *scratch, int64_t scratch_bytes, void *stream) {
    if (!head_stats || !input_grad || grad_rows <= 0 || grad_cols <= 0 || !weights || !weight_counts || num_weights <= 0 || num_weights > TAIL_MAX - 1 ||
        !out || !scratch || (prior && (prior_dim <= 0 || prior_dim > 5)) || scratch_bytes < qa_disc_step_tail_scratch_bytes() || ((uintptr_t)scratch & 15)) {
        snprintf(g_lerr, sizeof(g_lerr), "qa_disc_step_tail: bad argument (1..%d weight tensors, scratch >= qa_disc_step_tail_scratch_bytes(), zeroed once)", TAIL_MAX - 1);
        return QA_E_ARG; }
    TailArgs a{};
    a.t[0] = input_grad; a.n[0] = grad_rows * grad_cols;
    for (int i = 0; i < num_weights; ++i) {
        if (!weights[i] || weight_counts[i] <= 0) { snprintf(g_lerr, sizeof(g_lerr), "qa_disc_step_tail: empty weight tensor"); return QA_E_ARG; }
        a.t[1 + i] = weights[i]; a.n[1 + i] = weight_counts[i];
    }
    a.nt = 1 + num_weights; a.hs = head_stats; a.inv_rows = 1.0f / (float)grad_rows; a.out = out; a.acc = acc; a.step = step_counter; a.prior = prior; a.prior_dim = prior_dim; a.prior_c = prior_soft_coef;
    a.partial = (float *)scratch; a.ticket = (unsigned *)((float *)scratch + TAIL_MAX * TAIL_WG);
    hipLaunchKernelGGL(qa_disc_step_tail_kernel, dim3((unsigned)(a.nt * TAIL_WG)), dim3(256), 0, (hipStream_t)stream, a);
    hipError_t e = hipGetLastError();
    if (e != hipSuccess) { snprintf(g_lerr, sizeof(g_lerr), "qa_disc_step_tail: %s", hipGetErrorString(e)); return QA_E_DEVICE; }
    return QA_OK;
}

int qa_disc_prepare(const float *const *batches, const int64_t *rows, int32_t num_batches, int32_t dim, const float *task_mask,
                    const float *frame_mult, const float *task_weight_dev, const double *mean, const double *var, float epsilon, float clip,
                    float *out, void *stream) {
    if (!batches || !rows || !task_mask || !frame_mult || !out || num_batches <= 0 || num_batches > 3 || dim <= 0 || ((mean == nullptr) != (var == nullptr))) {
        snprintf(g_lerr, sizeof(g_lerr), "qa_disc_prepare: bad argument"); return QA_E_ARG; }
    PrepArgs a{};
    int64_t total = 0;
    for (int b = 0; b < num_batches; ++b) {
        if (!batches[b] || rows[b] <= 0) { snprintf(g_lerr, sizeof(g_lerr), "qa_disc_prepare: empty batch"); return QA_E_ARG; }
        a.src[b] = batches[b]; a.rows[b] = rows[b]; total += rows[b] * dim;
    }
    a.k = num_batches; a.dim = dim; a.task_mask = task_mask; a.frame_mult = frame_mult; a.task_w = task_weight_dev; a.mean = mean; a.var = var;
    a.eps = epsilon; a.clip = clip; a.out = out;
    hipLaunchKernelGGL(qa_disc_prepare_kernel, dim3((unsigned)((total + 255) / 256)), dim3(256), 0, (hipStream_t)stream, a);
    hipError_t e = hipGetLastError();
    if (e != hipSuccess) { snprintf(g_lerr, sizeof(g_lerr), "qa_disc_prepare: %s", hipGetErrorString(e)); return QA_E_DEVICE; }
    return QA_OK;
}

}
```

### quadrupedal_agility_amd/rsl_rl/algorithms/fused.py

```python
import ctypes as C
import os

import torch

from quadrupedal_agility_amd import _capi
from quadrupedal_agility_amd._capi import API, _ptr


ENABLED = True


def _f32c(t):
    return t if (t.dtype == torch.float32 and t.is_contiguous()) else t.contiguous().float()


class _PpoLoss(torch.autograd.Function):

    @staticmethod
    def forward(ctx, mu, std, value, actions, old_logp, old_mu, old_sigma, advantages, returns, target_values,
                clip, c_surr, c_value, c_bound, c_entropy, clipped_value):
        out, dmu, dstd, dvalue = ppo_loss_raw(mu, std, value, actions, old_logp, old_mu, old_sigma, advantages, returns, target_values, clip=clip, c_surr=c_surr,
                                              c_value=c_value, c_bound=c_bound, c_entropy=c_entropy, clipped_value=clipped_value)
        ctx.save_for_backward(dmu, dstd, dvalue)
        ctx.value_shape = value.shape
        ctx.std_shape = std.shape
        ctx.mark_non_differentiable(out)
        return out[0].clone(), out

    @staticmethod
    def backward(ctx, g_loss, _g_stats):
        dmu, dstd, dvalue = ctx.saved_tensors
        return (dmu * g_loss, (dstd * g_loss).view(ctx.std_shape), (dvalue * g_loss).view(ctx.value_shape),
                None, None, None, None, None, None, None, None, None, None, None, None, None)


def ppo_loss_raw(mu, std, value, actions, old_logp, old_mu, old_sigma, advantages, returns, target_values, *, clip, c_surr,
                 c_value, c_bound, c_entropy, clipped_value=True):
    mu_c, std_c, val_c = _f32c(mu.detach()), _f32c(std.detach()), _f32c(value.detach())
    fixed = [_f32c(x) for x in (actions, old_logp, old_mu, old_sigma, advantages, returns, target_values)]
    B = mu_c.shape[0]
    assert mu_c.is_cuda and mu_c.shape == (B, 12) and std_c.numel() == 12 and val_c.numel() == B
    dmu = torch.empty_like(mu_c)
    dstd = torch.empty(12, dtype=torch.float32, device=mu_c.device)
    dvalue = torch.empty(B, dtype=torch.float32, device=mu_c.device)
    out = torch.empty(8, dtype=torch.float32, device=mu_c.device)
    nscratch = int(API.lib.qa_ppo_loss_scratch_bytes(B))
    scratch = torch.empty(nscratch, dtype=torch.uint8, device=mu_c.device)
    API.launch("ppo_loss", _ptr(mu_c), _ptr(std_c), _ptr(val_c), *[_ptr(x) for x in fixed], B, 12, float(clip), float(c_surr),
               float(c_value), float(c_bound), float(c_entropy), int(bool(clipped_value)),
               _ptr(dmu), _ptr(dstd), _ptr(dvalue), _ptr(out), _ptr(scratch), nscratch, on=mu_c)
    return out, dmu, dstd, dvalue


def hybrid_ppo_loss_raw(logits, mean, std, value, actions, old_logp_d, old_logp_c, old_mu, old_sigma, advantages, returns, target_values, *,
                        clip, c_value, c_entropy, clipped_value=True):
    lg, mu_c, std_c, val_c = (_f32c(x.detach()) for x in (logits, mean, std, value))
    B, nd, nc = lg.shape[0], lg.shape[1], mu_c.shape[1]
    if (nd, nc) != (3, 18):
        return None
    fixed = [_f32c(x) for x in (actions, old_logp_d, old_logp_c, old_mu, old_sigma, advantages, returns, target_values)]
    assert fixed[0].shape == (B, 1 + nc) and val_c.numel() == B
    dev = lg.device
    dlogits, dmean = torch.empty_like(lg), torch.empty_like(mu_c)
    dstd, dvalue, out = torch.empty(nc, device=dev), torch.empty(B, device=dev), torch.empty(8, device=dev)
    n = int(API.lib.qa_hybrid_ppo_loss_scratch_bytes(B))
    scratch = torch.empty(n, dtype=torch.uint8, device=dev)
    API.launch("hybrid_ppo_loss", _ptr(lg), _ptr(mu_c), _ptr(std_c), _ptr(val_c), *[_ptr(x) for x in fixed], B, nd, nc, float(clip), float(c_value),
               float(c_entropy), int(bool(clipped_value)), _ptr(dlogits), _ptr(dmean), _ptr(dstd), _ptr(dvalue), _ptr(out), _ptr(scratch), n, on=dev)
    return out, dlogits, dmean, dstd, dvalue


_DEFER = [False]
_PENDING = {}
_RETIRED = []
_NO_DEFER = set()


def _retire(parts):
    if getattr(parts, "_qa_persistent", False):
        return
    if not torch.cuda.is_current_stream_capturing():
        parts.record_stream(torch.cuda.current_stream(parts.device))
    _RETIRED.append(parts)


class deferred_grad_finishes:
    def __enter__(self):
        self.prev = _DEFER[0]
        _DEFER[0] = ENABLED and os.environ.get("QA_DEFER_GRAD_FINISH", "1") != "0"
        del _RETIRED[:]
        _NO_DEFER.clear()
        return self

    def __exit__(self, *exc):
        _DEFER[0] = self.prev
        return False


def _defer_ok(param):
    if not (_DEFER[0] and param is not None and param.is_cuda and param.is_leaf and param.requires_grad):
# ... 137 lines not shown
    def backward(ctx, gv):
        (mask,) = ctx.saved_tensors
        _, gw = _masked_colsum(gv, mask)
        return None, gw.view(1, -1)


def mask_times_row(mask, w):
    if ENABLED and mask.is_cuda and torch.is_grad_enabled() and w.dim() == 2 and w.shape[0] == 1 and mask.dtype == torch.float32:
        return _MaskTimesRow.apply(mask, w)
    return mask * w


WGRAD_SLABS = 8


def weight_grad(g, x, param=None):
    rows, n = g.shape
    k = x.shape[1]
    S = WGRAD_SLABS
    if ENABLED and rows >= 8192 and rows % S == 0 and n * k >= 16384 and g.stride(1) == 1 and x.stride(1) == 1:
        slabs = torch.bmm(g.unflatten(0, (S, rows // S)).transpose(1, 2), x.unflatten(0, (S, rows // S)))
        if _defer_ok(param) and param.shape == (n, k) and param.is_contiguous():
            return _register_parts(param, slabs, S, n * k)
        return slab_sum(slabs)
    return g.t().mm(x)


class _NarrowLinear(torch.autograd.Function):

    @staticmethod
    def forward(ctx, x, weight, bias):
        ctx.save_for_backward(x, weight)
        return torch.addmm(bias, x, weight.t())

    @staticmethod
    def backward(ctx, gy):
        x, weight = ctx.saved_tensors
        _gradient_arriving(weight)
        gy = _f32c(gy)
        gx = gy.mm(weight) if ctx.needs_input_grad[0] else None
        if not (ctx.needs_input_grad[1] or ctx.needs_input_grad[2]):
            return gx, None, None
        xc = _f32c(x)
        rows, k = xc.shape
        o = weight.shape[0]
        gw = torch.empty_like(weight, memory_format=torch.contiguous_format)
        gb = torch.empty(o, dtype=torch.float32, device=x.device)
        n = int(API.lib.qa_narrow_wgrad_scratch_bytes(rows, o, k))
        scratch = torch.empty(n, dtype=torch.uint8, device=x.device)
        API.launch("narrow_wgrad", _ptr(gy), _ptr(xc), rows, o, k, _ptr(gw), _ptr(gb), _ptr(scratch), n, on=x)
        return gx, gw, gb


NARROW_MAX_OUT = 32
NARROW_MIN_ROWS = 1


def plain_linear(m, x):
    if (ENABLED and OWN_GEMM and x.is_cuda and torch.is_grad_enabled() and x.dim() == 2 and x.dtype == torch.float32 and m.bias is not None
            and m.out_features > NARROW_MAX_OUT and m.weight.requires_grad):
        return _MlpChain.apply(x, ((ACT_NONE, 0.0),), m.weight, m.bias)
    return narrow_linear(m, x)


def narrow_linear(m, x, always=False):
    if (ENABLED and x.is_cuda and torch.is_grad_enabled() and x.dim() == 2 and m.bias is not None and m.out_features <= NARROW_MAX_OUT
            and (x.shape[0] >= NARROW_MIN_ROWS or always) and x.dtype == torch.float32 and m.weight.requires_grad):
        return _NarrowLinear.apply(x, m.weight, m.bias)
    return m(x)


def linear_elu(x, weight, bias, alpha=1.0):
    return _LinearElu.apply(x, weight, bias, alpha)


def linear_act(x, weight, bias, code, alpha=1.0):
    if code == ACT_ELU:
        return _LinearElu.apply(x, weight, bias, alpha)
    return _MlpChain.apply(x, ((code, alpha),), weight, bias)


OWN_FWD_NARROW = os.environ.get("QA_OWN_FWD_NARROW", "0") == "1"
OWN_GEMM = os.environ.get("QA_OWN_GEMM", "1") != "0"
ACT_NONE, ACT_ELU, ACT_RELU = 0, 1, 2
ACT_TANH, ACT_LRELU, ACT_SELU, ACT_SIGMOID = _capi.MLP_ACT_TANH, _capi.MLP_ACT_LRELU, _capi.MLP_ACT_SELU, _capi.MLP_ACT_SIGMOID
NEW_ACTS = (ACT_TANH, ACT_LRELU, ACT_SELU, ACT_SIGMOID)
SELU_LAMBDA, SELU_ALPHA = 1.0507009873554805, 1.6732632423543772


def activation_code(m):
    nn = torch.nn
    if isinstance(m, nn.ELU):
        return ACT_ELU, float(m.alpha)
    if isinstance(m, nn.LeakyReLU):
        return (ACT_LRELU, 0.0) if m.negative_slope == 0.01 else None
    for cls, code in ((nn.ReLU, ACT_RELU), (nn.Tanh, ACT_TANH), (nn.SELU, ACT_SELU), (nn.Sigmoid, ACT_SIGMOID)):
        if type(m) is cls:
            return code, 0.0
    return None


def grad_code(code):
    return code + 3 if code else 0


def activation_derivative(code, y, alpha=1.0):
    if code == ACT_ELU:
        return torch.where(y > 0, torch.ones_like(y), y + alpha)
    if code == ACT_RELU:
        return (y > 0).to(y.dtype)
    if code == ACT_TANH:
        return 1.0 - y * y
    if code == ACT_LRELU:
        return torch.where(y > 0, torch.ones_like(y), torch.full_like(y, 0.01))
# ... 87 lines not shown


def pad16(k):
    return (int(k) + 15) // 16 * 16


def pad_k():
    return ENABLED and OWN_GEMM and (ALL_OWN or OWN_LAYERS == "all") and os.environ.get("QA_PAD_K", "1") != "0"


def slab_sum(parts):
    S = parts.shape[0]
    out = torch.empty(parts.shape[1:], dtype=torch.float32, device=parts.device)
    n = out.numel()
    API.launch("slab_sum", _ptr(parts), n, S, n, _ptr(out), on=parts)
    return out


class _MlpChain(torch.autograd.Function):

    @staticmethod
    def forward(ctx, x, spec, *params):
        h = _rows2d(x)
        acts = [h]
        kpad = h.shape[1] - params[0].shape[1]
        assert 0 <= kpad < 16, (h.shape, params[0].shape)
        w0 = torch.nn.functional.pad(params[0].detach(), (0, kpad)) if kpad else params[0]
        for i, (act, alpha) in enumerate(spec):
            h = linear_forward_raw(h, w0 if i == 0 else params[2 * i], params[2 * i + 1], act, alpha)
            acts.append(h)
        ctx.spec, ctx.kpad = spec, kpad
        ctx.save_for_backward(*acts, *params, *([w0] if kpad else []))
        return h

    @staticmethod
    def backward(ctx, gy):
        spec, kpad = ctx.spec, ctx.kpad
        L = len(spec)
        saved = ctx.saved_tensors
        acts, params = saved[:L + 1], saved[L + 1:L + 1 + 2 * L]
        _gradient_arriving(*params)
        w0p = saved[-1] if kpad else None
        g = _rows2d(gy)
        act_top, alpha_top = spec[-1]
        if act_top in NEW_ACTS:
            g = g * activation_derivative(act_top, acts[L])
        elif act_top != ACT_NONE:
            g, _ = _masked_colsum(g, acts[L]) if act_top == ACT_RELU else _elu_bwd(g, acts[L], alpha_top)
        grads = [None] * (2 * L)
        gx = None
        for i in range(L - 1, -1, -1):
            w = params[2 * i]
            need_w, need_b = ctx.needs_input_grad[2 + 2 * i], ctx.needs_input_grad[3 + 2 * i]
            if need_w or need_b:
                gw, gb = linear_backward_weight_raw(g, acts[i])
                if i == 0 and kpad:
                    gw = gw[:, :w.shape[1]].contiguous()
                grads[2 * i], grads[2 * i + 1] = (gw if need_w else None), (gb if need_b else None)
            if i > 0:
                g = linear_backward_input_raw(g, w, acts[i], spec[i - 1][0], spec[i - 1][1])
            elif ctx.needs_input_grad[0]:
                gx = linear_backward_input_raw(g, w0p if kpad else w, None, ACT_NONE)
        return (gx, None, *grads)


def _elu_bwd(gy, y, alpha):
    gy, y = _f32c(gy), _f32c(y)
    rows, cols = y.shape
    g = torch.empty_like(y)
    gb = torch.empty(cols, dtype=torch.float32, device=y.device)
    nscratch = int(API.lib.qa_elu_backward_bias_scratch_bytes(rows, cols))
    scratch = torch.empty(nscratch, dtype=torch.uint8, device=y.device)
    API.launch("elu_backward_bias", _ptr(gy), _ptr(y), _ptr(g), _ptr(gb), rows, cols, float(alpha), _ptr(scratch), nscratch, on=y)
    return g, gb


def _chain_spec(mods):
    out, i = [], 0
    while i < len(mods):
        m = mods[i]
        if not (isinstance(m, torch.nn.Linear) and m.bias is not None):
            return None
        nxt = mods[i + 1] if i + 1 < len(mods) else None
        ca = activation_code(nxt) if nxt is not None and not isinstance(nxt, torch.nn.Linear) else None
        if isinstance(nxt, torch.nn.ELU):
            out.append((m, ACT_ELU, float(nxt.alpha))); i += 2
        elif isinstance(nxt, torch.nn.ReLU):
            out.append((m, ACT_RELU, 0.0)); i += 2
        elif ca is not None:
            out.append((m, ca[0], ca[1])); i += 2
        else:
            out.append((m, ACT_NONE, 0.0)); i += 1
    return out if out and uniform_kinds(a for _, a, _ in out) else None


def _flatten(mods):
    flat = []
    for m in mods:
        flat.extend(list(m) if isinstance(m, torch.nn.Sequential) else [m])
    return flat


def mlp_chain(mods, x):
    flat = _flatten(mods)
    spec = _chain_spec(flat) if (ENABLED and OWN_GEMM and x.is_cuda and torch.is_grad_enabled() and x.dim() == 2 and x.dtype == torch.float32) else None
    if spec is None:
        for m in mods:
            if isinstance(m, torch.nn.Sequential):
                x = mlp_forward(m, x)
            elif isinstance(m, torch.nn.Linear):
                x = plain_linear(m, x)
            else:
                x = m(x)
        return x
    every = any(a in NEW_ACTS for _, a, _ in spec)
    i = 0
    while i < len(spec):
        m, act, alpha = spec[i]
        if every or own_layer(m.in_features, m.out_features):
            j = i
            while j < len(spec) and (every or own_layer(spec[j][0].in_features, spec[j][0].out_features)):
                j += 1
            params = []
            for mm, _, _ in spec[i:j]:
                params += [mm.weight, mm.bias]
            x = _MlpChain.apply(x, tuple((a, al) for _, a, al in spec[i:j]), *params)
            i = j
        else:
            x = linear_elu(x, m.weight, m.bias, alpha) if act == ACT_ELU else (_LinearRelu.apply(x, m.weight, m.bias) if act == ACT_RELU else plain_linear(m, x))
            i += 1
    return x


def mlp_forward(seq, x):
    mods = list(seq)
    if not (x.is_cuda and torch.is_grad_enabled()):
        return seq(x)
    if ENABLED and OWN_GEMM and x.dim() == 2 and x.dtype == torch.float32 and _chain_spec(mods) is not None:
        return mlp_chain(mods, x)
    i = 0
    while i < len(mods):
        m = mods[i]
        nxt = mods[i + 1] if i + 1 < len(mods) else None
        if isinstance(m, torch.nn.Linear) and isinstance(nxt, torch.nn.ELU) and m.bias is not None and x.dim() == 2:
            x = linear_elu(x, m.weight, m.bias, float(nxt.alpha))
            i += 2
        elif isinstance(m, torch.nn.Linear) and isinstance(nxt, torch.nn.ReLU) and m.bias is not None and x.dim() == 2:
            x = _LinearRelu.apply(x, m.weight, m.bias)
            i += 2
        elif isinstance(m, torch.nn.Linear):
            x = plain_linear(m, x)
            i += 1
        else:
            x = m(x)
            i += 1
    return x


ELEMENTWISE_ACTIVATIONS = (torch.nn.ELU, torch.nn.ReLU, torch.nn.Tanh, torch.nn.SELU, torch.nn.LeakyReLU, torch.nn.Sigmoid, torch.nn.GELU, torch.nn.SiLU,
                           torch.nn.Identity, torch.nn.Flatten)


def recordable(*nets):
    if not (ENABLED and OWN_GEMM):
        return False
    from quadrupedal_agility_amd.rsl_rl.modules.actor_critic import StateHistoryEncoder
    for net in nets:
        if net is None:
            continue
        for mod in net.modules():
            own = list(mod.parameters(recurse=False))
            if not any(p.requires_grad for p in own):
                continue
            if isinstance(mod, torch.nn.Linear):
# ... 93 lines not shown
        ctx.save_for_backward(grad)
        return out

    @staticmethod
    def backward(ctx, g):
        (grad,) = ctx.saved_tensors
        return grad * g, None, None


def pair_loss(a, b, mode):
    return _PairLoss.apply(a, b, mode)


def pair_loss_raw(a, b, mode):
    a = _f32c(a.detach())
    assert b.dtype == torch.float32 and b.stride(1) == 1 and a.shape == b.shape
    rows, cols = a.shape
    grad = torch.empty_like(a)
    out = torch.empty((), dtype=torch.float32, device=a.device)
    nscratch = int(API.lib.qa_pair_loss_scratch_bytes(rows))
    scratch = torch.empty(nscratch, dtype=torch.uint8, device=a.device)
    API.launch("pair_loss", _ptr(a), _ptr(b), rows, cols, b.stride(0), int(mode), _ptr(grad), _ptr(out), _ptr(scratch), nscratch, on=a)
    return out, grad


_pair_scratch = {}


def pair_losses_raw(jobs):
    n = len(jobs)
    recs = (_capi.QaPairJob * n)()
    outs, keep = [], []
    dev = jobs[0][0].device
    for i, (a, b, mode, scale) in enumerate(jobs):
        a = _f32c(a.detach())
        assert b.dtype == torch.float32 and b.stride(1) == 1 and a.shape == b.shape
        grad = torch.empty_like(a)
        out = torch.empty((), dtype=torch.float32, device=dev)
        if scale is not None:
            assert torch.is_tensor(scale) and scale.dtype == torch.float32 and scale.numel() == 1 and scale.device == dev
        r = recs[i]
        r.a, r.b, r.rows, r.cols, r.mode, r.b_stride = a.data_ptr(), b.data_ptr(), a.shape[0], a.shape[1], int(mode), b.stride(0)
        r.grad_scale, r.grad_a, r.out = (scale.data_ptr() if scale is not None else None), grad.data_ptr(), out.data_ptr()
        outs.append((out, grad)); keep.append(a)
    nb = int(API.lib.qa_pair_losses_scratch_bytes(C.cast(recs, C.c_void_p), n))
    key = (dev, nb)
    sc = _pair_scratch.get(key)
    if sc is None:
        sc = _pair_scratch[key] = torch.zeros(nb, dtype=torch.uint8, device=dev)
    API.launch("pair_losses", C.cast(recs, C.c_void_p), n, _ptr(sc), nb, on=dev)
    return outs


def accumulate_scalars(acc, scalars):
    n = len(scalars)
    if not (ENABLED and acc.is_cuda and acc.dtype == torch.float32 and acc.is_contiguous() and acc.numel() >= n and n <= 16
            and all(torch.is_tensor(x) and x.dtype == torch.float32 and x.numel() == 1 and x.device == acc.device for x in scalars)):
        acc[:n].add_(torch.stack([x.reshape(()) for x in scalars]))
        return
    API.launch("accumulate_scalars", _ptr(acc), (C.c_void_p * n)(*[x.data_ptr() for x in scalars]), n, on=acc)


def gather_rows(idx, srcs, dsts=None, block_dev=None):
    rows = idx.shape[-1]
    n = len(srcs)
    flat = [x if x.dim() == 2 else x.reshape(x.shape[0], -1) for x in srcs]
    assert idx.dtype == torch.int64 and idx.is_contiguous() and all(x.dtype == torch.float32 and x.stride(1) == 1 for x in flat)
    if dsts is None:
        dsts = [torch.empty(rows, x.shape[1], dtype=torch.float32, device=idx.device) for x in flat]
    src = (C.c_void_p * n)(*[x.data_ptr() for x in flat])
    dst = (C.c_void_p * n)(*[d.data_ptr() for d in dsts])
    strides = (C.c_int64 * n)(*[x.stride(0) for x in flat])
    widths = (C.c_int32 * n)(*[x.shape[1] for x in flat])
    API.launch("gather_rows", _ptr(idx), _ptr(block_dev) if block_dev is not None else None, rows, n, src, strides, widths, dst, on=idx)
    return dsts


def kl_lr_rule(kl, desired_kl, lr, factor=1.5, lr_min=1e-5, lr_max=1e-2):
    API.launch("kl_lr_rule", _ptr(kl), float(desired_kl), float(factor), float(lr_min), float(lr_max), _ptr(lr), on=lr)


def _take_pending(params):
    for p in params:
        e = _PENDING.pop(p.data_ptr(), None)
        if e is not None:
            _retire(e[1])


class ClipAdam:

    CHUNK = 2048
    SMALL_CHUNK = 32
    WIDE_PARTS = 16

    def __init__(self, optimizer, max_norm=None):
        self.opt = optimizer
        self.max_norm = float(max_norm) if max_norm else 0.0
        self._tab = None

    def _torch_step(self, params):
        if self.max_norm > 0:
            torch.nn.utils.clip_grad_norm_(params, self.max_norm)
        self.opt.step()

    def _build(self, items):
        opt = self.opt
        dev = items[0][0].device
        g0 = opt.param_groups[0]
        i64 = lambda xs: torch.tensor(xs, dtype=torch.int64, device=dev)
        st = [opt.state[p] for p, _ in items]
# ... 57 lines not shown
            if t["lr_val"] != float(lr):
                t["lr_dev"].fill_(float(lr)); t["lr_val"] = float(lr)
            lr_dev = t["lr_dev"]
        return dict(tab=t, params=params, ptrs=ptrs, pend=pend, lr_dev=lr_dev, inline=len(ptrs) <= 64)

    def step(self):
        pre = self._prepare()
        if pre is None:
            return
        if pre is False:
            opt = self.opt
            return self._torch_step([p for g in opt.param_groups for p in g["params"] if p.grad is not None])
        t, params, ptrs, pend, lr_dev, inline = pre["tab"], pre["params"], pre["ptrs"], pre["pend"], pre["lr_dev"], pre["inline"]
        if not inline and torch.cuda.is_current_stream_capturing():
            raise RuntimeError(f"ClipAdam: {len(ptrs)} gradient tensors (> 64) cannot ride in the kernel arguments, and the pointer-table "
                               "upload cannot be recorded into a hipGraph; this step stays eager")
        if not inline and ptrs != t["grad_ptrs"]:
            if t.get("copied") is not None:
                t["copied"].synchronize()
            t["grads_host"].copy_(torch.tensor(ptrs, dtype=torch.int64))
            t["grads"].copy_(t["grads_host"], non_blocking=True)
            t["copied"] = torch.cuda.Event()
            t["copied"].record()
            t["grad_ptrs"] = ptrs
        if pend is not None:
            n = len(params)
            src = (C.c_void_p * n)(*[(e[1].data_ptr() if e is not None else 0) for e in pend])
            stride = (C.c_int64 * n)(*[(e[3] if e is not None else 0) for e in pend])
            parts = (C.c_int32 * n)(*[(e[2] if e is not None else 0) for e in pend])
            try:
                API.launch("clip_adam_step_reduce", _ptr(t["params"]), (C.c_void_p * n)(*ptrs), _ptr(t["exp_avg"]), _ptr(t["exp_avg_sq"]), _ptr(t["steps"]), t["n"],
                           _ptr(t["chunk_tensor"]), _ptr(t["chunk_start"]), _ptr(t["chunk_len"]), t["num_chunks"], _ptr(t["wd"]),
                           _ptr(lr_dev), float(t["betas"][0]), float(t["betas"][1]), float(t["eps"]), self.max_norm,
                           _ptr(t["scratch"]), t["scratch"].numel(), src, stride, parts, on=params[0])
            finally:
                _take_pending(params)
            return
        name, garg = ("clip_adam_step_hostgrads", (C.c_void_p * len(ptrs))(*ptrs)) if inline else ("clip_adam_step", _ptr(t["grads"]))
        API.launch(name, _ptr(t["params"]), garg, _ptr(t["exp_avg"]), _ptr(t["exp_avg_sq"]), _ptr(t["steps"]), t["n"],
                   _ptr(t["chunk_tensor"]), _ptr(t["chunk_start"]), _ptr(t["chunk_len"]), t["num_chunks"], _ptr(t["wd"]),
                   _ptr(lr_dev), float(t["betas"][0]), float(t["betas"][1]), float(t["eps"]), self.max_norm,
                   _ptr(t["scratch"]), t["scratch"].numel(), on=params[0])


class ClipAdamPair:

    def __init__(self, first, second):
        self.first, self.second = first, second
        self._tab = None

    def warm(self):
        return self.step(dry=True)

    def step(self, kl=None, desired_kl=0.0, factor=1.5, lr_min=1e-5, lr_max=1e-2, dry=False):
        a, b = self.first, self.second
        self.why_not = None
        if not (ENABLED and a.max_norm > 0 and b.max_norm > 0):
            self.why_not = "an optimiser without clipping"
            return False
        ga, gb = a.opt.param_groups[0], b.opt.param_groups[0]
        if ga["betas"] != gb["betas"] or ga["eps"] != gb["eps"] or not (torch.is_tensor(gb["lr"]) and gb["lr"].dtype == torch.float32 and gb["lr"].is_cuda):
            self.why_not = "different betas / eps, or the second learning rate is not a device scalar"
            return False
        if kl is not None and not (torch.is_tensor(kl) and kl.is_cuda and kl.dtype == torch.float32 and kl.numel() == 1):
            self.why_not = "kl is not a device fp32 scalar"
            return False
        pa = a._prepare(for_pair=True)
        if not pa:
            self.why_not = f"the first optimiser cannot take the fused step ({pa})"
            return False
        pb = b._prepare(for_pair=True)
        if not pb or len(pa["ptrs"]) + len(pb["ptrs"]) > 64:
            self.why_not = f"the second optimiser cannot take the fused step ({pb if not pb else 'more than 64 tensors together'})"
            return False
        ta, tb = pa["tab"], pb["tab"]
        m = self._tab
        if m is None or m["ta"] is not ta or m["tb"] is not tb:
            if torch.cuda.is_current_stream_capturing():
                self.why_not = "the merged tables do not exist yet and a capture is running (call warm() first)"
                return False
            cat = lambda k: torch.cat([ta[k], tb[k]])
            m = self._tab = dict(ta=ta, tb=tb, params=cat("params"), exp_avg=cat("exp_avg"), exp_avg_sq=cat("exp_avg_sq"), steps=cat("steps"),
                                 chunk_tensor=torch.cat([ta["chunk_tensor"], tb["chunk_tensor"] + ta["n"]]), chunk_start=cat("chunk_start"), chunk_len=cat("chunk_len"),
                                 wd=cat("wd"), n=ta["n"] + tb["n"], num_chunks=ta["num_chunks"] + tb["num_chunks"],
                                 scratch=torch.zeros(ta["num_chunks"] + tb["num_chunks"] + 9, dtype=torch.float32, device=ta["params"].device))
        if dry:
            return True
        ptrs = pa["ptrs"] + pb["ptrs"]
        n = len(ptrs)
        pend = (pa["pend"] or [None] * len(pa["ptrs"])) + (pb["pend"] or [None] * len(pb["ptrs"]))
        src = (C.c_void_p * n)(*[(e[1].data_ptr() if e is not None else 0) for e in pend])
        stride = (C.c_int64 * n)(*[(e[3] if e is not None else 0) for e in pend])
        parts = (C.c_int32 * n)(*[(e[2] if e is not None else 0) for e in pend])
        pair = _capi.QaAdamPair(ta["n"], ta["num_chunks"], pb["lr_dev"].data_ptr(), b.max_norm, kl.data_ptr() if kl is not None else None,
                                float(desired_kl) if kl is not None else 0.0, float(factor), float(lr_min), float(lr_max))
        params = pa["params"] + pb["params"]
        try:
            API.launch("clip_adam_pair_step", _ptr(m["params"]), (C.c_void_p * n)(*ptrs), _ptr(m["exp_avg"]), _ptr(m["exp_avg_sq"]), _ptr(m["steps"]), m["n"],
                       _ptr(m["chunk_tensor"]), _ptr(m["chunk_start"]), _ptr(m["chunk_len"]), m["num_chunks"], _ptr(m["wd"]),
                       _ptr(pa["lr_dev"]), float(ta["betas"][0]), float(ta["betas"][1]), float(ta["eps"]), a.max_norm,
                       _ptr(m["scratch"]), m["scratch"].numel(), src, stride, parts, C.byref(pair), on=params[0])
        finally:
            _take_pending(params)
        return True


class StackedAdam:

    def __init__(self, optimizers, lib=None, prefix="qa_"):
        self.opts = list(optimizers)
        self.api = _capi.Api(lib, prefix)
        self._lr = {}
        self._ticket = None
        self._keep = None

    def _members(self):
        out = {}
        for k, o in enumerate(self.opts):
            for g in o.param_groups:
                for p in g["params"]:
                    out.setdefault(p, []).append((k, g))
        return out

    def ready(self):
        if not ENABLED or not self.opts or not all(type(o) is torch.optim.Adam for o in self.opts):
            return False
        g0 = self.opts[0].param_groups[0]
        mem = self._members()
        if len(mem) > _capi.ADAM_STACK_MAX_TENSORS or any(len(v) > _capi.ADAM_STACK_MAX_STATES for v in mem.values()):
            return False
        for o in self.opts:
            for g in o.param_groups:
                if g.get("amsgrad", False) or g.get("maximize", False) or g["betas"] != g0["betas"] or g["eps"] != g0["eps"]:
                    return False
                if torch.is_tensor(g["lr"]) and (g["lr"].dtype != torch.float32 or g["lr"].numel() != 1):
                    return False
                for p in g["params"]:
                    st = o.state.get(p, {})
                    if ("exp_avg" not in st or not torch.is_tensor(st["step"]) or st["step"].dtype != torch.float32 or st["step"].device != p.device
                            or p.dtype != torch.float32 or not p.is_contiguous()):
                        return False
        return True

    def _lr_dev(self, k, g, dev):
        lr = g["lr"]
        if torch.is_tensor(lr):
            return lr
        key = (k, id(g))
        e = self._lr.get(key)
        if e is None:
            e = self._lr[key] = [torch.zeros((), dtype=torch.float32, device=dev), None]
        if e[1] != float(lr):
            e[0].fill_(float(lr)); e[1] = float(lr)
        return e[0]

    def step(self, sources, reg=None):
# ... 504 lines not shown
```

### quadrupedal_agility_amd/rsl_rl/algorithms/gail.py

```python
import json
import os

import torch
import torch.nn as nn
import torch.nn.functional as F
import torch.optim as optim

from quadrupedal_agility_amd.rsl_rl import recording
from quadrupedal_agility_amd.rsl_rl.algorithms import fused as fused_mod
from quadrupedal_agility_amd.rsl_rl.algorithms.fused import ClipAdam, disc_loss, disc_prepare, ppo_loss
from quadrupedal_agility_amd.rsl_rl.storage import ReplayBuffer, RolloutStorage


def _vec11(out):
    return out if torch.is_tensor(out) else torch.stack(out)


class LossReadout:

    def __init__(self, dev_values):
        self._dev, self._host = dev_values, None

    def _values(self):
        if self._host is None:
# ... 224 lines not shown
                for k in range(n_d):
                    i_pi, i_lb, i_ulb = tabs[0][k], tabs[1][k], tabs[2][k]
                    acc_d += _vec11(self.update_ss_info_gail((rb.states[i_pi], rb.latent_eps[i_pi], rb.latent_c[i_pi]),
                                                                  (ml.preloaded_s_lb[i_lb], ml.preloaded_label[i_lb]), ml.preloaded_s_ulb[i_ulb]))
            else:
                gens = zip(self.disc_storage.feed_forward_generator(n_d, mb),
                           self.motion_loader.feed_forward_generator_lb(n_d, mb),
                           self.motion_loader.feed_forward_generator_ulb(n_d, mb))
                for s_pi, s_lb, s_ulb in gens:
                    acc_d += _vec11(self.update_ss_info_gail(s_pi, s_lb, s_ulb))
        self.storage.clear()
        self.priv_reg_counter += 1
        self._warm_updates += 1
        return LossReadout(torch.cat([acc_ac / n_ac, acc_d / n_d]))

    def _recordable_networks(self):
        other = (nn.SELU, nn.ReLU, nn.LeakyReLU, nn.Tanh, nn.Sigmoid, nn.GELU, nn.SiLU)
        plain = not any(isinstance(m, other) for net in (self.actor_critic, self.estimator) for m in net.modules())
        plain = plain or (fused_mod.OWN_GEMM and fused_mod.uniform_activation(self.actor_critic, self.estimator) is not None)
        disc_ok = (not self.amp_enabled) or (self.disc._relu_trunk() is not None and self.disc_loss_function == "MSELoss")
        return bool(fused_mod.ENABLED and plain and disc_ok)

    def _clamp_std(self):
        if not self.actor_critic.fixed_std and self.min_std is not None:
            self.actor_critic.std.data.clamp_(min=self.min_std)

    def _priv_reg_coef_now(self):
        s0, s1, t0, t1 = self.priv_reg_coef_schedual
        stage = min(max(self.priv_reg_counter - t0, 0) / t1, 1)
        return stage * (s1 - s0) + s0

    def _ac_updates_recorded(self, perm=None):
        dev, st = self.device, self.storage
        batch = st.num_envs * st.num_transitions_per_env
        mb = batch // self.num_mini_batches
        nmb = self.num_mini_batches
        if self._ac_graph is None:
            try:
                self._acc_ac = torch.zeros(6, device=dev)
                self._priv_coef_dev = torch.zeros((), device=dev)
                flat = [x.flatten(0, 1) for x in (st.observations, st.actions, st.values, st.advantages, st.returns,
                                                  st.actions_log_prob, st.mu, st.sigma)]
                if (fused_mod.pad_k() or self._train_chain_rows(mb) is not None) and getattr(st, "_obs_padded", None) is not None:
                    flat[0] = st._obs_padded.flatten(0, 1)
                sync = self.grad_sync
                all_params = list(self.estimator.parameters()) + list(self.actor_critic.parameters())

                self._hist_latent_all = torch.zeros(batch, self.num_latent, device=dev)
                self._hist_cols = slice(self.num_prop + self.num_explicit + self.num_latent,
                                        self.num_prop + self.num_explicit + self.num_latent + self.num_hist * self.num_prop)
                self._gather_srcs = flat + [self._hist_latent_all]
                self._perm_bufs = [torch.empty(nmb * mb, x.shape[1] if x.dim() == 2 else 1, device=dev) for x in self._gather_srcs]

                def front(i):
                    obs, act, val, adv, ret, logp, mu, sig, hl = (b[i * mb:(i + 1) * mb] for b in self._perm_bufs)
                    return self._ac_forward_backward((obs, obs, act, val, adv, ret, logp, mu, sig, (None, None), None, hl))

                torch.cuda.synchronize()
                for o in (self.optim_ac, self.optim_estimator):
                    o.zero_grad(set_to_none=True)
                self._recording_ac = True
                graphs = []
                pool = torch.cuda.graph_pool_handle()
                try:
                    epoch_graph = sync is None and self._train_chain_rows(mb) is not None and os.environ.get("QA_STEP_UNROLL", "1") != "0"

                    def slot(i):
                        stats, kl = front(i)
                        self._ac_apply(kl)
                        fused_mod.accumulate_scalars(self._acc_ac, stats)

                    def epoch():
                        for i in range(nmb):
                            slot(i)
                            for o in (self.optim_ac, self.optim_estimator):
                                o.zero_grad(set_to_none=True)

                    if epoch_graph:
                        graphs.append((recording.record(epoch, pool=pool)[0], None, None))
                    for i in range(0 if epoch_graph else nmb):
                        if sync is None:
                            graphs.append((recording.record(lambda: slot(i), pool=pool)[0], None, None))
                        else:
                            graphs.append(recording.record_data_parallel(lambda: front(i)[::-1], self._ac_apply, self._acc_ac, all_params, sync.world, pool))
                        for o in (self.optim_ac, self.optim_estimator):
                            o.zero_grad(set_to_none=True)
                    self._ac_graph = graphs
                finally:
                    self._recording_ac = False
            except Exception as e:
                recording.capture_failed("ppo update graph", e)
                self._ac_graph = False
                acc = torch.zeros(6, device=dev)
                for sample in st.mini_batch_generator(self.num_mini_batches, self.num_learning_epochs):
                    acc += torch.stack(self.update_actor_critic(sample))
                return acc
        self._priv_coef_dev.fill_(float(self._priv_reg_coef_now()))
        self._acc_ac.zero_()
        with torch.no_grad():
            self._hist_latent_all.copy_(self.actor_critic.infer_hist_latent(st.observations.flatten(0, 1)[:, self._hist_cols]))
        if perm is None:
            perm = torch.randperm(nmb * mb, device=dev)
        fused_mod.gather_rows(perm, self._gather_srcs, dsts=self._perm_bufs)
        for _ in range(self.num_learning_epochs):
            for ga, gb, bucket in self._ac_graph:
                recording.replay_step(ga, gb, bucket, self.grad_sync)
        return self._acc_ac.clone()

    def _disc_updates_recorded(self, n_steps, mb, tables=None):
        dev = self.device
        if self._disc_graph is None:
            try:
                self._n_samples_dev = torch.zeros((), device=dev)
                self._acc_d = torch.zeros(11, device=dev)
                ml, rb = self.motion_loader, self.disc_storage
                n_lb, n_ulb = ml.preloaded_s_lb.shape[0], ml.preloaded_s_ulb.shape[0]

                self._d_tables = [torch.zeros(n_steps, mb, dtype=torch.int64, device=dev) for _ in range(4)]
                self._d_step = torch.zeros((), dtype=torch.int64, device=dev)
                flat2 = lambda x: x.reshape(x.shape[0], -1)

                def one_step():
                    t_pi, t_lb, t_ulb, t_lab = self._d_tables
# ... 22 lines not shown
                        self._acc_d.add_(_vec11(out))
                        self._d_step.add_(1)
                self._n_samples_dev.fill_(float(rb.num_samples))
                self._info_max_dev.fill_(float(self.info_max_coef_on))
                torch.cuda.synchronize()
                for o in (self.optim_d, self.optim_q_eps, self.optim_q_c):
                    o.zero_grad(set_to_none=True)
                if self._disc_stream is None:
                    self._disc_stream = torch.cuda.Stream(device=dev)
                self._recording_disc = True
                try:
                    unroll = max((k for k in (8, 5, 4, 2, 1) if n_steps % k == 0), default=1) if os.environ.get("QA_STEP_UNROLL", "1") != "0" else 1

                    def steps():
                        for _ in range(unroll):
                            one_step()
                    g, _ = recording.record(steps, stream=self._disc_stream)
                finally:
                    self._recording_disc = False
                self._disc_graph, self._disc_unroll, self._disc_graph_steps = g, unroll, n_steps
            except Exception as e:
                recording.capture_failed("disc update graph", e)
                self._disc_graph = False
                acc = torch.zeros(11, device=dev)
                gens = zip(self.disc_storage.feed_forward_generator(n_steps, mb), self.motion_loader.feed_forward_generator_lb(n_steps, mb),
                           self.motion_loader.feed_forward_generator_ulb(n_steps, mb))
                for s_pi, s_lb, s_ulb in gens:
                    acc += _vec11(self.update_ss_info_gail(s_pi, s_lb, s_ulb))
                return acc
        self._n_samples_dev.fill_(float(self.disc_storage.num_samples))
        self._info_max_dev.fill_(float(self.info_max_coef_on))
        if self._task_w_dev is not None:
            self._task_w_dev.fill_(float(self.env.task_obs_weight))
        self._acc_d.zero_()
        ml = self.motion_loader
        t_pi, t_lb, t_ulb, t_lab = self._d_tables
        if tables is not None:
            t_pi.copy_(tables["pi"]); t_lb.copy_(tables["lb"]); t_ulb.copy_(tables["ulb"])
        else:
            t_pi.copy_((torch.rand(t_pi.shape, device=dev) * self._n_samples_dev).long())
            torch.randint(0, ml.preloaded_s_lb.shape[0], t_lb.shape, device=dev, out=t_lb)
            torch.randint(0, ml.preloaded_s_ulb.shape[0], t_ulb.shape, device=dev, out=t_ulb)
        t_lab.copy_(ml.preloaded_label[t_lb.view(-1)].view(t_lb.shape))
        self._d_step.zero_()
        assert n_steps == self._disc_graph_steps
        for _ in range(n_steps // self._disc_unroll):
            self._disc_graph.replay()
        return self._acc_d

    def _sync_grads(self, params):
        if self.grad_sync is not None:
            self.grad_sync(params)

    def _ac_forward_backward(self, sample):
        (obs, critic_obs, actions, target_values, advantages, returns, old_logp, old_mu, old_sigma, _hid, _masks) = sample[:11]
        hist_latent = sample[11] if len(sample) > 11 else None
        ac = self.actor_critic
        fused = self._on_gpu and self.use_fused_loss
        if fused and not ac.fixed_std:
            return self._ac_forward_backward_direct(obs, critic_obs, actions, target_values, advantages, returns, old_logp, old_mu, old_sigma, hist_latent)
        if fused:
            mu = ac._actor_mean(obs.detach(), False)
            value = ac.evaluate(critic_obs.detach())
            ppo, stats = ppo_loss(mu, ac.std, value, actions, old_logp, old_mu, old_sigma, advantages, returns, target_values,
                                  clip=self.clip_param, c_surr=self.surrogate_loss_coef, c_value=self.value_loss_coef,
                                  c_bound=self.bounds_loss_coef, c_entropy=self.entropy_coef, clipped_value=self.use_clipped_value_loss)
        else:
            ac.update_distribution(obs.detach(), False)
            logp = ac.get_actions_log_prob(actions)
            value = ac.evaluate(critic_obs.detach())
            mu, sigma, entropy = ac.action_mean, ac.action_std, ac.entropy

        a = self.num_prop; b = a + self.num_explicit; c = b + self.num_latent; d = c + self.num_hist * self.num_prop
        obs_prop, obs_explicit, obs_latent, obs_hist = obs[:, :a], obs[:, a:b], obs[:, b:c], obs[:, c:d]
        priv_latent = ac.infer_priv_latent(obs_latent)
        if hist_latent is None:
            with torch.no_grad():
                hist_latent = ac.infer_hist_latent(obs_hist)
        if fused:
            priv_reg_loss = fused_mod.pair_loss(priv_latent, hist_latent, fused_mod.PAIR_ROW_L2)
        else:
            priv_reg_loss = (priv_latent - hist_latent).norm(p=2, dim=1).mean()
        priv_reg_coef = self._priv_coef_dev if self._recording_ac else self._priv_reg_coef_now()

        if fused:
            estimator_loss = fused_mod.pair_loss(self.estimator(obs_prop), obs_explicit, fused_mod.PAIR_MSE)
        else:
            estimator_loss = (self.estimator(obs_prop) - obs_explicit).pow(2).mean()
        self.optim_estimator.zero_grad()
        estimator_loss.backward()

        adaptive = self.desired_kl is not None and self.schedule == "adaptive"
        kl_mean = None
        if adaptive:
            with torch.no_grad():
                if fused:
                    kl_mean = stats[5]
                else:
                    kl = torch.sum(torch.log(sigma / old_sigma + 1.0e-5) +
                                   (torch.square(old_sigma) + torch.square(old_mu - mu)) / (2.0 * torch.square(sigma)) - 0.5, dim=-1)
                    kl_mean = kl.mean()

        if fused:
            surrogate_loss, value_loss, b_mean, ent_mean = stats[1], stats[2], stats[3], stats[4]
            loss = ppo + priv_reg_coef * priv_reg_loss
        else:
            adv = torch.squeeze(advantages)
            ratio = torch.exp(logp - torch.squeeze(old_logp))
            surrogate_loss = torch.max(-adv * ratio, -adv * torch.clamp(ratio, 1.0 - self.clip_param, 1.0 + self.clip_param)).mean()
            if self.use_clipped_value_loss:
                v_clip = target_values + (value - target_values).clamp(-self.clip_param, self.clip_param)
                value_loss = torch.max((value - returns).pow(2), (v_clip - returns).pow(2)).mean()
            else:
                value_loss = (returns - value).pow(2).mean()
            b_loss = (torch.clamp(mu + 1.0, max=0.0) ** 2 + torch.clamp(mu - 1.0, min=0.0) ** 2).sum(dim=-1)
            b_mean, ent_mean = b_loss.mean(), entropy.mean()
            loss = (self.surrogate_loss_coef * surrogate_loss + self.value_loss_coef * value_loss +
                    self.bounds_loss_coef * b_mean - self.entropy_coef * ent_mean + priv_reg_coef * priv_reg_loss)
        self.optim_ac.zero_grad()
        loss.backward()
        return (surrogate_loss.detach(), value_loss.detach(), b_mean.detach(), ent_mean.detach(),
                priv_reg_loss.detach(), estimator_loss.detach()), kl_mean

    def _ac_forward_backward_direct(self, obs, critic_obs, actions, target_values, advantages, returns, old_logp, old_mu, old_sigma, hist_latent):
        ac = self.actor_critic
        a = self.num_prop; b = a + self.num_explicit; c = b + self.num_latent; d = c + self.num_hist * self.num_prop
        priv_reg_coef = self._priv_coef_dev if self._recording_ac else self._priv_reg_coef_now()
        chain = self._train_chain(obs, critic_obs)
        self._chain_sides = None
        if chain is not None:
            return self._ac_forward_backward_chain(chain, obs, actions, target_values, advantages, returns, old_logp, old_mu, old_sigma, hist_latent, priv_reg_coef)
        cur = torch.cuda.current_stream()
        if self.branch_streams and self._branch is None:
            self._branch = (torch.cuda.Stream(device=self.device), torch.cuda.Stream(device=self.device))
        s_critic, s_small = self._branch if self.branch_streams else (cur, cur)
        if self.branch_streams:
            s_critic.wait_stream(cur); s_small.wait_stream(cur)
        self.optim_estimator.zero_grad()
        self.optim_ac.zero_grad()
        with torch.cuda.stream(s_critic):
            value = ac.evaluate(critic_obs.detach())
        with torch.cuda.stream(s_small):
            priv_latent = ac.infer_priv_latent(obs[:, b:c])
            if hist_latent is None:
                with torch.no_grad():
                    hist_latent = ac.infer_hist_latent(obs[:, c:d])
            est = self.estimator(obs[:, :a])
            if torch.is_tensor(priv_reg_coef) and priv_reg_coef.dtype == torch.float32 and priv_reg_coef.device == obs.device and os.environ.get("QA_PAIR_LOSSES", "1") != "0":
                (priv_reg_loss, g_priv), (estimator_loss, g_est) = fused_mod.pair_losses_raw(
                    [(priv_latent, hist_latent, fused_mod.PAIR_ROW_L2, priv_reg_coef), (est, obs[:, a:b], fused_mod.PAIR_MSE, None)])
            else:
                priv_reg_loss, g_priv = fused_mod.pair_loss_raw(priv_latent, hist_latent, fused_mod.PAIR_ROW_L2)
                g_priv = g_priv * priv_reg_coef
                estimator_loss, g_est = fused_mod.pair_loss_raw(est, obs[:, a:b], fused_mod.PAIR_MSE)
        mu = ac._actor_mean(obs.detach(), False)
        if self.branch_streams:
            cur.wait_stream(s_critic)
        out, dmu, dstd, dvalue = fused_mod.ppo_loss_raw(mu, ac.std, value, actions, old_logp, old_mu, old_sigma, advantages, returns, target_values,
                                                        clip=self.clip_param, c_surr=self.surrogate_loss_coef, c_value=self.value_loss_coef,
                                                        c_bound=self.bounds_loss_coef, c_entropy=self.entropy_coef,
                                                        clipped_value=self.use_clipped_value_loss)
        if self.branch_streams:
            cur.wait_stream(s_small)
            if not self._recording_ac:
                for t in (value, priv_latent, est, g_priv, g_est):
                    t.record_stream(cur)
        if self._recording_ac:
            fused_mod.assert_recordable_graph([est, mu, value, priv_latent], "PPO step")
        with fused_mod.deferred_grad_finishes():
            torch.autograd.backward([est, mu, value, priv_latent], [g_est, dmu, dvalue.view_as(value), g_priv])
        if self.grad_sync is not None:
            fused_mod.flush_pending_grads()
        ac.std.grad = dstd.view_as(ac.std)
        adaptive = self.desired_kl is not None and self.schedule == "adaptive"
        return (out[1], out[2], out[3], out[4], priv_reg_loss, estimator_loss), (out[5] if adaptive else None)

    def _disc_train_chain(self, rows, n_u):
        from quadrupedal_agility_amd.rsl_rl.algorithms import train_chain
        if not (train_chain.ENABLED and train_chain.DISC_ENABLED) or rows > train_chain.MAX_ROWS:
            return None
        cache = self.__dict__.setdefault("_disc_train_chains", {})
        if (rows, n_u) not in cache:
            cache[(rows, n_u)] = train_chain.DiscTrainChain.describe(self.disc, rows, n_u) or False
        return cache[(rows, n_u)] or None

    def _train_chain(self, obs, critic_obs):
        if obs.data_ptr() != critic_obs.data_ptr() or obs.stride(1) != 1:
            return None
        return self._train_chain_rows(obs.shape[0])

    def _train_chain_rows(self, rows):
        from quadrupedal_agility_amd.rsl_rl.algorithms import train_chain
        if not (train_chain.ENABLED and self._on_gpu and self.use_fused_loss) or rows > train_chain.MAX_ROWS or self.actor_critic.fixed_std:
            return None
        cache = self.__dict__.setdefault("_train_chains", {})
        if rows not in cache:
            cache[rows] = train_chain.PpoTrainChain.describe(self.actor_critic, self.estimator, rows) or False
        return cache[rows] or None

    def _ac_forward_backward_chain(self, chain, obs, actions, target_values, advantages, returns, old_logp, old_mu, old_sigma, hist_latent, priv_reg_coef):
        ac = self.actor_critic
        a = self.num_prop; b = a + self.num_explicit; c = b + self.num_latent; d = c + self.num_hist * self.num_prop
        self.optim_estimator.zero_grad()
        self.optim_ac.zero_grad()
        chain.pack()
        est, mu, value, priv_latent = chain.forward(obs)
        if hist_latent is None:
            with torch.no_grad():
                hist_latent = ac.infer_hist_latent(obs[:, c:d])
        if torch.is_tensor(priv_reg_coef) and priv_reg_coef.dtype == torch.float32 and priv_reg_coef.device == obs.device and os.environ.get("QA_PAIR_LOSSES", "1") != "0":
            (priv_reg_loss, g_priv), (estimator_loss, g_est) = fused_mod.pair_losses_raw(
                [(priv_latent, hist_latent, fused_mod.PAIR_ROW_L2, priv_reg_coef), (est, obs[:, a:b], fused_mod.PAIR_MSE, None)])
        else:
            priv_reg_loss, g_priv = fused_mod.pair_loss_raw(priv_latent, hist_latent, fused_mod.PAIR_ROW_L2)
            g_priv = g_priv * priv_reg_coef
            estimator_loss, g_est = fused_mod.pair_loss_raw(est, obs[:, a:b], fused_mod.PAIR_MSE)
        out, dmu, dstd, dvalue = fused_mod.ppo_loss_raw(mu, ac.std, value, actions, old_logp, old_mu, old_sigma, advantages, returns, target_values,
                                                        clip=self.clip_param, c_surr=self.surrogate_loss_coef, c_value=self.value_loss_coef,
                                                        c_bound=self.bounds_loss_coef, c_entropy=self.entropy_coef,
                                                        clipped_value=self.use_clipped_value_loss)
        chain.backward(g_est, dmu, dvalue, g_priv)
        self._chain_sides = chain.sides if self.grad_sync is None else None
        if self.grad_sync is not None:
            fused_mod.flush_pending_grads()
        ac.std.grad = dstd.view_as(ac.std)
        adaptive = self.desired_kl is not None and self.schedule == "adaptive"
        return (out[1], out[2], out[3], out[4], priv_reg_loss, estimator_loss), (out[5] if adaptive else None)

    def _ac_apply(self, kl_mean):
        sides = getattr(self, "_chain_sides", None)
        if sides is not None:
            with sides.fork(0):
                self._step_estimator.step()
        elif (self._step_pair is not None and self.use_fused_loss and (kl_mean is None or (kl_mean.dtype == torch.float32 and kl_mean.is_contiguous()))
              and self._step_pair.step(kl_mean, self.desired_kl)):
            if fused_mod.pending_grads():
                fused_mod.flush_pending_grads()
            return
        else:
            self._step_estimator.step()
        if kl_mean is not None:
            self._apply_kl_schedule(kl_mean)
        self._step_ac.step()
        if sides is not None:
            sides.join()
        if fused_mod.pending_grads():
            fused_mod.flush_pending_grads()

    def update_actor_critic(self, sample):
        stats, kl_mean = self._ac_forward_backward(sample)
        if self.grad_sync is not None:
            params = list(self.estimator.parameters()) + list(self.actor_critic.parameters())
            synced = self.grad_sync(params, extra=[kl_mean] if kl_mean is not None else None)
            if kl_mean is not None:
                kl_mean = synced[0].reshape(())
        self._ac_apply(kl_mean)
        return stats

    def _apply_kl_schedule(self, kl_mean):
        tgt = self.desired_kl
        if self._on_gpu and self.use_fused_loss and kl_mean.dtype == torch.float32 and kl_mean.is_contiguous():
            fused_mod.kl_lr_rule(kl_mean, tgt, self._lr_ac)
        elif self._on_gpu:
            lr = self._lr_ac
            down = torch.clamp(lr / 1.5, min=1e-5)
            up = torch.clamp(lr * 1.5, max=1e-2)
            new = torch.where(kl_mean > tgt * 2.0, down, torch.where((kl_mean < tgt / 2.0) & (kl_mean > 0.0), up, lr))
            lr.copy_(new)
        else:
            k = float(kl_mean)
            if k > tgt * 2.0:
                self._lr_ac = max(1e-5, self._lr_ac / 1.5)
            elif tgt / 2.0 > k > 0.0:
                self._lr_ac = min(1e-2, self._lr_ac * 1.5)
            for g in self.optim_ac.param_groups:
                g["lr"] = self._lr_ac

    def _fused_prep_ok(self, width):
        nm = self.disc_normalizer
        return bool(self._on_gpu and self.use_fused_loss and nm is not None and hasattr(nm, "count") and torch.is_tensor(getattr(nm, "mean", None))
                    and self.disc.disc_obs_len * self.disc.num_disc_obs == width)

    def _task_weight_dev(self):
        w = getattr(self.env, "task_obs_weight_dev", None)
        if w is None:
            if self._task_w_dev is None:
                self._task_w_dev = torch.ones((), device=self.device)
            if not torch.cuda.is_current_stream_capturing():
                self._task_w_dev.fill_(float(self.env.task_obs_weight))
            w = self._task_w_dev
        return w

    def update_ss_info_gail(self, sample_disc_policy, sample_disc_expert_lb, sample_disc_expert_ulb, acc=None, step=None, prepared=None):
        self._tail_folded = False
        policy_state, policy_eps, policy_c = sample_disc_policy
        expert_lb, label_lb = sample_disc_expert_lb
        expert_ulb = sample_disc_expert_ulb
        w = getattr(self.env, "task_obs_weight_dev", None)
        fused_prep = prepared is None and self._fused_prep_ok(policy_state.shape[-1])
        if prepared is not None:
            x_all, nl, npi = prepared
            expert_lb, policy_state, expert_ulb = x_all[:nl], x_all[nl:nl + npi], x_all[nl + npi:]
        elif fused_prep:
# ... 244 lines not shown
```

Measured before the change: 3.084 million.

## Defer PPO loss finish into the Adam step and fold scalar accumulation

Splits the fused PPO loss into a partials kernel and a deferred finish. The finish is then run inside the Adam sum-of-squares kernel, by the block that owns the std tensor's first chunk. Scalar stat accumulation is folded into the Adam finalize kernel, and dedicated single-output head forward/backward kernels are added. The aim is to cut kernel launches per minibatch in the PPO update loop. The cost is cross-kernel coupling, more complex pending-state handling, and an ordering dependency where dstd must be ready before the std grad is read.

Measured after the change: 3.111 million, median of 2. About the same (+0.9%).

```diff
diff --git a/__graft_entry__.py b/__graft_entry__.py
--- a/__graft_entry__.py
+++ b/__graft_entry__.py
@@ -42,6 +42,7 @@
     srcs.append(os.path.join(ROOT, "include", "qa_sim_curriculum.h"))
     srcs.append(os.path.join(ROOT, "include", "qa_tsc_curriculum.h"))
     srcs.append(os.path.join(ROOT, "include", "qa_sim_rewards.h"))
+    srcs.append(os.path.join(ROOT, "include", "qa_learner_ext.h"))
     return srcs
 
 
diff --git a/include/qa_learner_ext.h b/include/qa_learner_ext.h
--- /dev/null
+++ b/include/qa_learner_ext.h
@@ -0,0 +1,47 @@
+#ifndef QA_LEARNER_EXT_H
+#define QA_LEARNER_EXT_H
+
+#include "qa_sim.h"
+
+#ifdef __cplusplus
+extern "C" {
+#endif
+
+int qa_ppo_loss_partials(const float *mu, const float *std, const float *value, const float *actions, const float *old_logp,
+                         const float *old_mu, const float *old_sigma, const float *advantages, const float *returns,
+                         const float *target_values, int64_t B, int32_t num_actions, float clip, float c_surr, float c_value,
+                         float c_bound, float c_entropy, int32_t clipped_value, float *dmu, float *dvalue,
+                         void *scratch, int64_t scratch_bytes, void *stream);
+int qa_ppo_finish(const float *partials, int64_t B, float c_surr, float c_value, float c_bound, float c_entropy, float *out,
+                  float *dstd, void *stream);
+
+typedef struct qa_ppo_pending {
+    const float *partials;
+    int64_t B;
+    float c_surr, c_value, c_bound, c_entropy;
+    float *out;
+    float *dstd;
+} qa_ppo_pending;
+
+typedef struct qa_step_scalars {
+    float *acc;
+    const float *src[QA_ACC_MAX];
+    int32_t count;
+} qa_step_scalars;
+
+int qa_clip_adam_pair_step_pending(float *const *params, const float *const *grads_host, float *const *exp_avg, float *const *exp_avg_sq,
+                                   float *const *steps, int32_t num_tensors, const int32_t *chunk_tensor, const int32_t *chunk_start,
+                                   const int32_t *chunk_len, int32_t num_chunks, const float *weight_decay, const float *lr, float beta1,
+                                   float beta2, float eps, float max_norm, float *scratch, int64_t scratch_floats,
+                                   const float *const *red_src_host, const int64_t *red_stride_host, const int32_t *red_parts_host,
+                                   const qa_adam_pair *pair, const qa_ppo_pending *pending, const qa_step_scalars *scalars, void *stream);
+
+int qa_head1_forward(const float *x, int64_t ldx, const float *w, const float *b, float *y, int64_t rows, int32_t K, void *stream);
+int64_t qa_head1_backward_scratch_bytes(int64_t rows, int32_t K);
+int qa_head1_backward(const float *gy, const float *x, int64_t ldx, const float *w, float *gx, int64_t rows, int32_t K,
+                      float *grad_weight, float *grad_bias, void *scratch, int64_t scratch_bytes, void *stream);
+
+#ifdef __cplusplus
+}
+#endif
+#endif
diff --git a/quadrupedal_agility_amd/_capi.py b/quadrupedal_agility_amd/_capi.py
--- a/quadrupedal_agility_amd/_capi.py
+++ b/quadrupedal_agility_amd/_capi.py
@@ -236,7 +236,31 @@
     f = getattr(lib, prefix + "set_terrain_curriculum"); f.argtypes = [C.c_void_p] * 4 + [C.c_int32, C.c_int32, C.c_float, C.c_float]; f.restype = C.c_int
     f = getattr(lib, prefix + "tsc_obstacle_curriculum"); f.argtypes = [C.POINTER(QaTscObstCurr), C.c_void_p]; f.restype = C.c_int
     f = getattr(lib, prefix + "set_extra_rewards"); f.argtypes = [C.c_void_p, C.POINTER(QaExtraRewards)]; f.restype = C.c_int
+    f = getattr(lib, prefix + "ppo_loss_partials")
+    f.argtypes = [C.c_void_p] * 10 + [C.c_int64, C.c_int32] + [C.c_float] * 5 + [C.c_int32] + [C.c_void_p] * 3 + [C.c_int64, C.c_void_p]
+    f.restype = C.c_int
+    f = getattr(lib, prefix + "ppo_finish"); f.argtypes = [C.c_void_p, C.c_int64] + [C.c_float] * 4 + [C.c_void_p] * 3; f.restype = C.c_int
+    f = getattr(lib, prefix + "clip_adam_pair_step_pending")
+    f.argtypes = [C.c_void_p] * 5 + [C.c_int32] + [C.c_void_p] * 3 + [C.c_int32, C.c_void_p, C.c_void_p] + [C.c_float] * 4 + [C.c_void_p, C.c_int64] + [C.c_void_p] * 7
+    f.restype = C.c_int
+    f = getattr(lib, prefix + "head1_forward"); f.argtypes = [C.c_void_p, C.c_int64, C.c_void_p, C.c_void_p, C.c_void_p, C.c_int64, C.c_int32, C.c_void_p]; f.restype = C.c_int
+    f = getattr(lib, prefix + "head1_backward_scratch_bytes"); f.argtypes = [C.c_int64, C.c_int32]; f.restype = C.c_int64
+    f = getattr(lib, prefix + "head1_backward")
+    f.argtypes = [C.c_void_p, C.c_void_p, C.c_int64, C.c_void_p, C.c_void_p, C.c_int64, C.c_int32, C.c_void_p, C.c_void_p, C.c_void_p, C.c_int64, C.c_void_p]
+    f.restype = C.c_int
     return lib
+
+
+ACC_MAX = 16
+
+
+class QaPpoPending(C.Structure):
+    _fields_ = [("partials", C.c_void_p), ("B", C.c_int64), ("c_surr", C.c_float), ("c_value", C.c_float), ("c_bound", C.c_float), ("c_entropy", C.c_float),
+                ("out", C.c_void_p), ("dstd", C.c_void_p)]
+
+
+class QaStepScalars(C.Structure):
+    _fields_ = [("acc", C.c_void_p), ("src", C.c_void_p * ACC_MAX), ("count", C.c_int32)]
 
 
 class QaExtraRewards(C.Structure):
@@ -367,7 +391,8 @@
 ABI_SYMBOLS = ["arena_bytes", "create", "destroy", "tensor_info", "env_step", "env_step_dev", "reset_all", "simulate",
                "set_mocap", "debug_post_physics", "env_physics_step", "tsc_reset", "tsc_reset_dev", "simulate_if", "gae", "ppo_loss", "ppo_loss_scratch_bytes", "hybrid_ppo_loss", "hybrid_ppo_loss_scratch_bytes", "elu_backward_bias",
                "elu_backward_bias_scratch_bytes", "narrow_wgrad", "narrow_wgrad_scratch_bytes", "linear_forward", "linear_backward_input", "linear_backward_weight", "linear_backward_weight_scratch_bytes", "linear_backward_weight_layout", "linear_backward_weight_batch", "linear_backward_weight_batch_layout", "linear_backward_weight_batch_scratch_bytes", "slab_sum", "linear_forward_split", "linear_forward_split_scratch_bytes", "depth_stem_forward", "depth_stem_backward", "depth_stem_backward_scratch_bytes", "conv_nhwc_forward", "conv_nhwc_backward_input", "conv_nhwc_backward_weight", "conv_nhwc_backward_weight_scratch_bytes", "elu_backward_pad", "normalizer_update", "normalizer_apply", "clip_adam_step", "clip_adam_step_hostgrads", "clip_adam_step_reduce", "clip_adam_pair_step", "grad_reduce", "adam_stack_step", "rollout_act", "rollout_act_store", "rollout_act_hybrid", "rollout_post", "rollout_post_amp", "disc_loss", "disc_loss_logits", "disc_loss_scratch_bytes", "disc_prepare", "disc_sample_prepare", "disc_step_tail", "disc_step_tail_scratch_bytes", "pair_loss", "pair_loss_scratch_bytes", "pair_losses", "pair_losses_scratch_bytes", "accumulate_scalars", "gather_rows", "kl_lr_rule", "episode_means", "set_lean_exports", "mlp_packed_floats", "mlp_pack", "mlp_forward", "mlp_strands", "mlp_groups", "mlp_set_groups", "tsc_set_commands", "tsc_goal_step", "tsc_observations", "tsc_depth_update", "tsc_reset_stats", "tsc_push", "tsc_start_pose", "tsc_reset_where", "last_error", "abi_version"]
-EXTENSION_SYMBOLS = ["set_terrain_curriculum", "tsc_obstacle_curriculum", "set_extra_rewards"]
+EXTENSION_SYMBOLS = ["set_terrain_curriculum", "tsc_obstacle_curriculum", "set_extra_rewards",
+                     "ppo_loss_partials", "ppo_finish", "clip_adam_pair_step_pending", "head1_forward", "head1_backward_scratch_bytes", "head1_backward"]
 
 _LIB = None
 LIB_PATH = os.environ.get("QA_LIB") or os.path.join(os.path.dirname(os.path.abspath(__file__)), "csrc", "libqa_sim.so")
diff --git a/quadrupedal_agility_amd/csrc/qa_learner.hip b/quadrupedal_agility_amd/csrc/qa_learner.hip
--- a/quadrupedal_agility_amd/csrc/qa_learner.hip
+++ b/quadrupedal_agility_amd/csrc/qa_learner.hip
@@ -4,6 +4,7 @@
 
 #include "../../include/qa_sim.h"
 #include "../../include/qa_tsc_curriculum.h"
+#include "../../include/qa_learner_ext.h"
 #include "qa_device.h"
 
 namespace {
@@ -104,8 +105,8 @@
     }
 }
 
-__global__ void __launch_bounds__(256) qa_ppo_finish_kernel(const float *partial, int nblocks, int64_t B, float c_surr, float c_value,
-                                                            float c_bound, float c_entropy, float *out, float *dstd) {
+__device__ __forceinline__ void ppo_finish_block(const float *partial, int nblocks, int64_t B, float c_surr, float c_value,
+                                                 float c_bound, float c_entropy, float *out, float *dstd) {
     constexpr int LANES = 256 / PPO_SUMS;
     __shared__ double s_acc[256];
     __shared__ double s_tot[PPO_SUMS];
@@ -127,6 +128,10 @@
     if (t == 5) out[0] = (float)((c_surr * s_tot[0] + c_value * s_tot[1] + c_bound * s_tot[2] - c_entropy * s_tot[3]) * invB);
     if (t == 6 || t == 7) out[t] = 0.f;
     if (t >= 8 && t < 8 + PPO_D) dstd[t - 8] = (float)(s_tot[5 + t - 8] * invB);
+}
+__global__ void __launch_bounds__(256) qa_ppo_finish_kernel(const float *partial, int nblocks, int64_t B, float c_surr, float c_value,
+                                                            float c_bound, float c_entropy, float *out, float *dstd) {
+    ppo_finish_block(partial, nblocks, B, c_surr, c_value, c_bound, c_entropy, out, dstd);
 }
 
 constexpr int HYB_ND = 3, HYB_NC = 18, HYB_SUMS = 5 + HYB_NC;
@@ -528,7 +533,7 @@
     return acc;
 }
 
-__global__ void __launch_bounds__(256) qa_adam_sumsq_kernel(AdamArgs a) {
+__device__ __forceinline__ void adam_sumsq_block(const AdamArgs &a) {
     __shared__ float s_w[4];
     __shared__ float s_q[256];
     const int c = blockIdx.x, t = a.chunk_tensor[c];
@@ -545,8 +550,20 @@
     __syncthreads();
     if (threadIdx.x == 0) a.scratch[4 + c] = (s_w[0] + s_w[1]) + (s_w[2] + s_w[3]);
 }
-
-__global__ void __launch_bounds__(256) qa_adam_finalize_kernel(AdamArgs a) {
+__global__ void __launch_bounds__(256) qa_adam_sumsq_kernel(AdamArgs a) { adam_sumsq_block(a); }
+
+struct PendArgs { const float *partial; int nblocks; int64_t B; float c_surr, c_value, c_bound, c_entropy; float *out, *dstd; int std_tensor; };
+__global__ void __launch_bounds__(256) qa_adam_sumsq_pending_kernel(AdamArgs a, PendArgs p) {
+    const int c = blockIdx.x;
+    if (a.chunk_tensor[c] == p.std_tensor && a.chunk_start[c] == 0) {
+        ppo_finish_block(p.partial, p.nblocks, p.B, p.c_surr, p.c_value, p.c_bound, p.c_entropy, p.out, p.dstd);
+        __threadfence_block();
+        __syncthreads();
+    }
+    adam_sumsq_block(a);
+}
+
+__device__ __forceinline__ void adam_finalize_block(const AdamArgs &a) {
     __shared__ double s_acc[256], s_acc2[256];
     const int split = a.split_chunk > 0 ? a.split_chunk : a.num_chunks;
     double acc = 0.0, acc2 = 0.0;
@@ -585,6 +602,7 @@
         }
     }
 }
+__global__ void __launch_bounds__(256) qa_adam_finalize_kernel(AdamArgs a) { adam_finalize_block(a); }
 
 constexpr int PAIR_BLOCK = 256;
 
@@ -742,6 +760,12 @@
 __global__ void qa_accumulate_scalars_kernel(AccArgs a) {
     const int i = threadIdx.x;
     if (i < a.n) a.acc[i] += a.src[i][0];
+}
+
+__global__ void __launch_bounds__(256) qa_adam_finalize_stats_kernel(AdamArgs a, AccArgs s) {
+    adam_finalize_block(a);
+    if (threadIdx.x == 0)
+        for (int i = 0; i < s.n; ++i) s.acc[i] += s.src[i][0];
 }
 
 __global__ void qa_kl_lr_rule_kernel(const float *kl, float desired_kl, float factor, float lr_min, float lr_max, float *lr) {
@@ -1365,6 +1389,85 @@
     if (j < io.rows[0] && io.label_src) io.label_out[j] = io.label_src[blk * io.rows[0] + j];
 }
 
+constexpr int HEAD1_ROWS = 64, HEAD1_TILE = 128;
+
+__global__ void __launch_bounds__(256) qa_head1_forward_kernel(const float *__restrict__ x, int64_t ldx, const float *__restrict__ w, const float *__restrict__ b,
+                                                               float *__restrict__ y, int64_t rows, int K) {
+    const int c = threadIdx.x & 31, q = threadIdx.x >> 5;
+    const int64_t r0 = (int64_t)blockIdx.x * HEAD1_ROWS + 8 * q;
+    float acc[8];
+#pragma unroll
+    for (int j = 0; j < 8; ++j) acc[j] = 0.f;
+    for (int k0 = 0; k0 < K; k0 += HEAD1_TILE) {
+        const int k = k0 + 4 * c;
+        const bool on = k < K;
+        const float4 zero = make_float4(0.f, 0.f, 0.f, 0.f);
+        const float4 w4 = on ? *(const float4 *)(w + k) : zero;
+        float4 v[8];
+#pragma unroll
+        for (int j = 0; j < 8; ++j) v[j] = (on && r0 + j < rows) ? *(const float4 *)(x + (r0 + j) * ldx + k) : zero;
+#pragma unroll
+        for (int j = 0; j < 8; ++j) acc[j] = fmaf(v[j].w, w4.w, fmaf(v[j].z, w4.z, fmaf(v[j].y, w4.y, fmaf(v[j].x, w4.x, acc[j]))));
+    }
+#pragma unroll
+    for (int j = 0; j < 8; ++j)
+#pragma unroll
+        for (int o = 16; o > 0; o >>= 1) acc[j] += __shfl_xor(acc[j], o, 64);
+    float mine = acc[0];
+#pragma unroll
+    for (int j = 1; j < 8; ++j) mine = c == j ? acc[j] : mine;
+    if (c < 8 && r0 + c < rows) y[r0 + c] = mine + b[0];
+}
+
+__global__ void __launch_bounds__(256) qa_head1_backward_kernel(const float *__restrict__ gy, const float *__restrict__ x, int64_t ldx, const float *__restrict__ w,
+                                                                float *__restrict__ gx, int64_t rows, int K, float *__restrict__ partial) {
+    __shared__ float4 s_p[8][32];
+    __shared__ float s_g[8];
+    const int c = threadIdx.x & 31, q = threadIdx.x >> 5;
+    const int64_t r0 = (int64_t)blockIdx.x * HEAD1_ROWS + 8 * q;
+    float *out = partial + (int64_t)blockIdx.x * (K + 1);
+    float g[8];
+#pragma unroll
+    for (int j = 0; j < 8; ++j) g[j] = r0 + j < rows ? gy[r0 + j] : 0.f;
+    for (int k0 = 0; k0 < K; k0 += HEAD1_TILE) {
+        const int k = k0 + 4 * c;
+        const bool on = k < K;
+        const float4 zero = make_float4(0.f, 0.f, 0.f, 0.f);
+        const float4 w4 = on ? *(const float4 *)(w + k) : zero;
+        float4 v[8];
+#pragma unroll
+        for (int j = 0; j < 8; ++j) v[j] = (on && r0 + j < rows) ? *(const float4 *)(x + (r0 + j) * ldx + k) : zero;
+        float4 a = zero;
+#pragma unroll
+        for (int j = 0; j < 8; ++j) {
+            if (on && r0 + j < rows) *(float4 *)(gx + (r0 + j) * (int64_t)K + k) = make_float4(g[j] * w4.x, g[j] * w4.y, g[j] * w4.z, g[j] * w4.w);
+            a.x = fmaf(g[j], v[j].x, a.x); a.y = fmaf(g[j], v[j].y, a.y); a.z = fmaf(g[j], v[j].z, a.z); a.w = fmaf(g[j], v[j].w, a.w);
+        }
+        s_p[q][c] = a;
+        __syncthreads();
+        if (q == 0 && on) {
+            float4 t = s_p[0][c];
+#pragma unroll
+            for (int z = 1; z < 8; ++z) { const float4 u = s_p[z][c]; t.x += u.x; t.y += u.y; t.z += u.z; t.w += u.w; }
+            out[k] = t.x; out[k + 1] = t.y; out[k + 2] = t.z; out[k + 3] = t.w;
+        }
+        __syncthreads();
+    }
+    if (c == 0) {
+        float t = g[0];
+#pragma unroll
+        for (int j = 1; j < 8; ++j) t += g[j];
+        s_g[q] = t;
+    }
+    __syncthreads();
+    if (threadIdx.x == 0) {
+        float t = s_g[0];
+#pragma unroll
+        for (int z = 1; z < 8; ++z) t += s_g[z];
+        out[K] = t;
+    }
+}
+
 }
 
 extern thread_local char qa_err_buf[512];
@@ -1373,26 +1476,53 @@
 extern "C" {
 
 int64_t qa_ppo_loss_scratch_bytes(int64_t B) { return B <= 0 ? -1 : (int64_t)sizeof(float) * PPO_SUMS * ((B + PPO_BLOCK - 1) / PPO_BLOCK); }
+
+static int ppo_loss_launch(const char *who, bool finish, const float *mu, const float *std, const float *value, const float *actions, const float *old_logp,
+                           const float *old_mu, const float *old_sigma, const float *advantages, const float *returns,
+                           const float *target_values, int64_t B, int32_t num_actions, float clip, float c_surr, float c_value,
+                           float c_bound, float c_entropy, int32_t clipped_value, float *dmu, float *dstd, float *dvalue, float *out,
+                           void *scratch, int64_t scratch_bytes, void *stream) {
+    if (!mu || !std || !value || !actions || !old_logp || !old_mu || !old_sigma || !advantages || !returns || !target_values ||
+        !dmu || (finish && (!dstd || !out)) || !dvalue || !scratch || B <= 0) { snprintf(g_lerr, sizeof(g_lerr), "%s: null pointer or empty batch", who); return QA_E_ARG; }
+    if (num_actions != PPO_D) { snprintf(g_lerr, sizeof(g_lerr), "%s: num_actions must be %d", who, PPO_D); return QA_E_ARG; }
+    if ((((uintptr_t)mu | (uintptr_t)actions | (uintptr_t)old_mu | (uintptr_t)old_sigma | (uintptr_t)dmu) & 15) != 0) {
+        snprintf(g_lerr, sizeof(g_lerr), "%s: (B,12) tensors must be 16-byte aligned", who); return QA_E_ARG; }
+    hipStream_t st = (hipStream_t)stream;
+    const int blocks = (int)((B + PPO_BLOCK - 1) / PPO_BLOCK);
+    if (scratch_bytes < qa_ppo_loss_scratch_bytes(B)) { snprintf(g_lerr, sizeof(g_lerr), "%s: scratch too small", who); return QA_E_ARG; }
+    PpoArgs a{mu, std, value, actions, old_logp, old_mu, old_sigma, advantages, returns, target_values, dmu, dvalue, (float *)scratch,
+              B, clip, c_surr, c_value, c_bound, c_entropy, clipped_value};
+    hipLaunchKernelGGL(qa_ppo_loss_kernel, dim3(blocks), dim3(PPO_BLOCK), 0, st, a);
+    if (finish) hipLaunchKernelGGL(qa_ppo_finish_kernel, dim3(1), dim3(256), 0, st, (const float *)scratch, blocks, B, c_surr, c_value, c_bound, c_entropy, out, dstd);
+    hipError_t e = hipGetLastError();
+    if (e != hipSuccess) { snprintf(g_lerr, sizeof(g_lerr), "%s: %s", who, hipGetErrorString(e)); return QA_E_DEVICE; }
+    return QA_OK;
+}
 
 int qa_ppo_loss(const float *mu, const float *std, const float *value, const float *actions, const float *old_logp,
                 const float *old_mu, const float *old_sigma, const float *advantages, const float *returns,
                 const float *target_values, int64_t B, int32_t num_actions, float clip, float c_surr, float c_value,
                 float c_bound, float c_entropy, int32_t clipped_value, float *dmu, float *dstd, float *dvalue, float *out,
                 void *scratch, int64_t scratch_bytes, void *stream) {
-    if (!mu || !std || !value || !actions || !old_logp || !old_mu || !old_sigma || !advantages || !returns || !target_values ||
-        !dmu || !dstd || !dvalue || !out || !scratch || B <= 0) { snprintf(g_lerr, sizeof(g_lerr), "qa_ppo_loss: null pointer or empty batch"); return QA_E_ARG; }
-    if (num_actions != PPO_D) { snprintf(g_lerr, sizeof(g_lerr), "qa_ppo_loss: num_actions must be %d", PPO_D); return QA_E_ARG; }
-    if ((((uintptr_t)mu | (uintptr_t)actions | (uintptr_t)old_mu | (uintptr_t)old_sigma | (uintptr_t)dmu) & 15) != 0) {
-        snprintf(g_lerr, sizeof(g_lerr), "qa_ppo_loss: (B,12) tensors must be 16-byte aligned"); return QA_E_ARG; }
-    hipStream_t st = (hipStream_t)stream;
+    return ppo_loss_launch("qa_ppo_loss", true, mu, std, value, actions, old_logp, old_mu, old_sigma, advantages, returns, target_values, B, num_actions, clip,
+                           c_surr, c_value, c_bound, c_entropy, clipped_value, dmu, dstd, dvalue, out, scratch, scratch_bytes, stream);
+}
+
+int qa_ppo_loss_partials(const float *mu, const float *std, const float *value, const float *actions, const float *old_logp,
+                         const float *old_mu, const float *old_sigma, const float *advantages, const float *returns,
+                         const float *target_values, int64_t B, int32_t num_actions, float clip, float c_surr, float c_value,
+                         float c_bound, float c_entropy, int32_t clipped_value, float *dmu, float *dvalue,
+                         void *scratch, int64_t scratch_bytes, void *stream) {
+    return ppo_loss_launch("qa_ppo_loss_partials", false, mu, std, value, actions, old_logp, old_mu, old_sigma, advantages, returns, target_values, B, num_actions,
+                           clip, c_surr, c_value, c_bound, c_entropy, clipped_value, dmu, nullptr, dvalue, nullptr, scratch, scratch_bytes, stream);
+}
+
+int qa_ppo_finish(const float *partials, int64_t B, float c_surr, float c_value, float c_bound, float c_entropy, float *out, float *dstd, void *stream) {
+    if (!partials || !out || !dstd || B <= 0) { snprintf(g_lerr, sizeof(g_lerr), "qa_ppo_finish: null pointer or empty batch"); return QA_E_ARG; }
     const int blocks = (int)((B + PPO_BLOCK - 1) / PPO_BLOCK);
-    if (scratch_bytes < qa_ppo_loss_scratch_bytes(B)) { snprintf(g_lerr, sizeof(g_lerr), "qa_ppo_loss: scratch too small"); return QA_E_ARG; }
-    PpoArgs a{mu, std, value, actions, old_logp, old_mu, old_sigma, advantages, returns, target_values, dmu, dvalue, (float *)scratch,
-              B, clip, c_surr, c_value, c_bound, c_entropy, clipped_value};
-    hipLaunchKernelGGL(qa_ppo_loss_kernel, dim3(blocks), dim3(PPO_BLOCK), 0, st, a);
-    hipLaunchKernelGGL(qa_ppo_finish_kernel, dim3(1), dim3(256), 0, st, (const float *)scratch, blocks, B, c_surr, c_value, c_bound, c_entropy, out, dstd);
-    hipError_t e = hipGetLastError();
-    if (e != hipSuccess) { snprintf(g_lerr, sizeof(g_lerr), "qa_ppo_loss: %s", hipGetErrorString(e)); return QA_E_DEVICE; }
+    hipLaunchKernelGGL(qa_ppo_finish_kernel, dim3(1), dim3(256), 0, (hipStream_t)stream, partials, blocks, B, c_surr, c_value, c_bound, c_entropy, out, dstd);
+    hipError_t e = hipGetLastError();
+    if (e != hipSuccess) { snprintf(g_lerr, sizeof(g_lerr), "qa_ppo_finish: %s", hipGetErrorString(e)); return QA_E_DEVICE; }
     return QA_OK;
 }
 
@@ -1500,7 +1630,8 @@
                             float *const *exp_avg_sq, float *const *steps, int32_t num_tensors, const int32_t *chunk_tensor, const int32_t *chunk_start,
                             const int32_t *chunk_len, int32_t num_chunks, const float *weight_decay, const float *lr, float beta1, float beta2, float eps,
                             float max_norm, float *scratch, int64_t scratch_floats, void *stream, const char *who,
-                            const float *const *red_src = nullptr, const int64_t *red_stride = nullptr, const int32_t *red_parts = nullptr, const qa_adam_pair *pair = nullptr) {
+                            const float *const *red_src = nullptr, const int64_t *red_stride = nullptr, const int32_t *red_parts = nullptr, const qa_adam_pair *pair = nullptr,
+                            const qa_ppo_pending *pending = nullptr, const qa_step_scalars *scalars = nullptr) {
     if (!params || (!grads_dev && !grads_host) || !exp_avg || !exp_avg_sq || !steps || !chunk_tensor || !chunk_start || !chunk_len || !weight_decay || !lr ||
         !scratch || num_tensors <= 0 || num_chunks <= 0 || scratch_floats < 4 + (int64_t)num_chunks || (grads_host && num_tensors > QA_ADAM_MAX_INLINE)) {
         snprintf(g_lerr, sizeof(g_lerr), "%s: bad argument", who); return QA_E_ARG; }
@@ -1527,8 +1658,30 @@
             if (red_parts[t] > 0) a.has_reduce = 1;
         }
     }
+    PendArgs pd{};
+    if (pending) {
+        if (!pair || !pending->partials || !pending->out || !pending->dstd || pending->B <= 0) { snprintf(g_lerr, sizeof(g_lerr), "%s: bad pending objective", who); return QA_E_ARG; }
+        int std_t = -1;
+        for (int t = 0; t < num_tensors; ++t) if (grads_host[t] == pending->dstd) std_t = t;
+        if (std_t < 0 || a.red_parts[std_t] > 0) {
+            snprintf(g_lerr, sizeof(g_lerr), "%s: the pending objective's dstd must be one of the step's gradient tensors, not in parts", who); return QA_E_ARG; }
+        pd = PendArgs{pending->partials, (int)((pending->B + PPO_BLOCK - 1) / PPO_BLOCK), pending->B, pending->c_surr, pending->c_value, pending->c_bound,
+                      pending->c_entropy, pending->out, pending->dstd, std_t};
+    }
+    AccArgs sc{};
+    if (scalars) {
+        if (!pair || !scalars->acc || scalars->count <= 0 || scalars->count > QA_ACC_MAX) { snprintf(g_lerr, sizeof(g_lerr), "%s: 1..%d logged scalars expected", who, QA_ACC_MAX); return QA_E_ARG; }
+        sc.acc = scalars->acc; sc.n = scalars->count;
+        for (int i = 0; i < scalars->count; ++i) { if (!scalars->src[i]) { snprintf(g_lerr, sizeof(g_lerr), "%s: null scalar source %d", who, i); return QA_E_ARG; } sc.src[i] = scalars->src[i]; }
+    }
     hipStream_t st = (hipStream_t)stream;
-    if (!(max_norm > 0.f) && scratch_floats >= 5 + (int64_t)num_chunks) {
+    if (pair && (pending || scalars)) {
+        if (pending) hipLaunchKernelGGL(qa_adam_sumsq_pending_kernel, dim3(num_chunks), dim3(256), 0, st, a, pd);
+        else hipLaunchKernelGGL(qa_adam_sumsq_kernel, dim3(num_chunks), dim3(256), 0, st, a);
+        if (scalars) hipLaunchKernelGGL(qa_adam_finalize_stats_kernel, dim3(1), dim3(256), 0, st, a, sc);
+        else hipLaunchKernelGGL(qa_adam_finalize_kernel, dim3(1), dim3(256), 0, st, a);
+        hipLaunchKernelGGL(qa_adam_update_kernel<false>, dim3(num_chunks), dim3(256), 0, st, a);
+    } else if (!(max_norm > 0.f) && scratch_floats >= 5 + (int64_t)num_chunks) {
         hipLaunchKernelGGL(qa_adam_update_kernel<true>, dim3(num_chunks), dim3(256), 0, st, a);
     } else {
         if (max_norm > 0.f) hipLaunchKernelGGL(qa_adam_sumsq_kernel, dim3(num_chunks), dim3(256), 0, st, a);
@@ -1997,4 +2150,51 @@
     return QA_OK;
 }
 
-}
+int qa_clip_adam_pair_step_pending(float *const *params, const float *const *grads_host, float *const *exp_avg, float *const *exp_avg_sq,
+                                   float *const *steps, int32_t num_tensors, const int32_t *chunk_tensor, const int32_t *chunk_start,
+                                   const int32_t *chunk_len, int32_t num_chunks, const float *weight_decay, const float *lr, float beta1,
+                                   float beta2, float eps, float max_norm, float *scratch, int64_t scratch_floats,
+                                   const float *const *red_src_host, const int64_t *red_stride_host, const int32_t *red_parts_host,
+                                   const qa_adam_pair *pair, const qa_ppo_pending *pending, const qa_step_scalars *scalars, void *stream) {
+    if (!pair) { snprintf(g_lerr, sizeof(g_lerr), "qa_clip_adam_pair_step_pending: bad argument"); return QA_E_ARG; }
+    return clip_adam_launch(params, nullptr, grads_host, exp_avg, exp_avg_sq, steps, num_tensors, chunk_tensor, chunk_start, chunk_len, num_chunks, weight_decay,
+                            lr, beta1, beta2, eps, max_norm, scratch, scratch_floats, stream, "qa_clip_adam_pair_step_pending", red_src_host, red_stride_host,
+                            red_parts_host, pair, pending, scalars);
+}
+
+static int head1_check(const char *who, const float *x, int64_t ldx, const float *w, int64_t rows, int32_t K) {
+    if (!x || !w || rows <= 0 || K <= 0 || (K & 3) || ldx < K || (ldx & 3) || (((uintptr_t)x | (uintptr_t)w) & 15) || (rows + HEAD1_ROWS - 1) / HEAD1_ROWS > 0x7fffffff) {
+        snprintf(g_lerr, sizeof(g_lerr), "%s: x (rows, K) and w 16-byte aligned with K %% 4 == 0, ldx %% 4 == 0 and ldx >= K expected", who); return QA_E_ARG; }
+    return QA_OK;
+}
+
+int qa_head1_forward(const float *x, int64_t ldx, const float *w, const float *b, float *y, int64_t rows, int32_t K, void *stream) {
+    if (head1_check("qa_head1_forward", x, ldx, w, rows, K) != QA_OK) return QA_E_ARG;
+    if (!b || !y) { snprintf(g_lerr, sizeof(g_lerr), "qa_head1_forward: null pointer"); return QA_E_ARG; }
+    const int nb = (int)((rows + HEAD1_ROWS - 1) / HEAD1_ROWS);
+    hipLaunchKernelGGL(qa_head1_forward_kernel, dim3(nb), dim3(256), 0, (hipStream_t)stream, x, ldx, w, b, y, rows, (int)K);
+    hipError_t e = hipGetLastError();
+    if (e != hipSuccess) { snprintf(g_lerr, sizeof(g_lerr), "qa_head1_forward: %s", hipGetErrorString(e)); return QA_E_DEVICE; }
+    return QA_OK;
+}
+
+int64_t qa_head1_backward_scratch_bytes(int64_t rows, int32_t K) {
+    return (rows <= 0 || K <= 0) ? -1 : (int64_t)sizeof(float) * ((rows + HEAD1_ROWS - 1) / HEAD1_ROWS) * ((int64_t)K + 1);
+}
+
+int qa_head1_backward(const float *gy, const float *x, int64_t ldx, const float *w, float *gx, int64_t rows, int32_t K,
+                      float *grad_weight, float *grad_bias, void *scratch, int64_t scratch_bytes, void *stream) {
+    if (head1_check("qa_head1_backward", x, ldx, w, rows, K) != QA_OK) return QA_E_ARG;
+    if (!gy || !gx || !scratch || ((uintptr_t)gx & 15) || (grad_weight == nullptr) != (grad_bias == nullptr)) {
+        snprintf(g_lerr, sizeof(g_lerr), "qa_head1_backward: null pointer, gx not 16-byte aligned, or only one of grad_weight / grad_bias"); return QA_E_ARG; }
+    if (scratch_bytes < qa_head1_backward_scratch_bytes(rows, K)) { snprintf(g_lerr, sizeof(g_lerr), "qa_head1_backward: scratch too small"); return QA_E_ARG; }
+    hipStream_t st = (hipStream_t)stream;
+    const int nb = (int)((rows + HEAD1_ROWS - 1) / HEAD1_ROWS);
+    hipLaunchKernelGGL(qa_head1_backward_kernel, dim3(nb), dim3(256), 0, st, gy, x, ldx, w, gx, rows, (int)K, (float *)scratch);
+    if (grad_weight) hipLaunchKernelGGL(qa_colsum_finish2_kernel, dim3((K + 1 + 31) / 32), dim3(256), 0, st, (const float *)scratch, nb, (int)K + 1, (int)K, grad_weight, grad_bias);
+    hipError_t e = hipGetLastError();
+    if (e != hipSuccess) { snprintf(g_lerr, sizeof(g_lerr), "qa_head1_backward: %s", hipGetErrorString(e)); return QA_E_DEVICE; }
+    return QA_OK;
+}
+
+}
diff --git a/quadrupedal_agility_amd/rsl_rl/algorithms/fused.py b/quadrupedal_agility_amd/rsl_rl/algorithms/fused.py
--- a/quadrupedal_agility_amd/rsl_rl/algorithms/fused.py
+++ b/quadrupedal_agility_amd/rsl_rl/algorithms/fused.py
@@ -34,8 +34,22 @@
                 None, None, None, None, None, None, None, None, None, None, None, None, None)
 
 
+class PpoPending:
+
+    def __init__(self, partials, B, coefs, out, dstd):
+        self.partials, self.B, self.coefs, self.out, self.dstd, self.done = partials, B, coefs, out, dstd, False
+
+    def struct(self):
+        return _capi.QaPpoPending(self.partials.data_ptr(), self.B, *self.coefs, self.out.data_ptr(), self.dstd.data_ptr())
+
+    def finish(self):
+        if not self.done:
+            API.launch("ppo_finish", _ptr(self.partials), self.B, *self.coefs, _ptr(self.out), _ptr(self.dstd), on=self.out)
+            self.done = True
+
+
 def ppo_loss_raw(mu, std, value, actions, old_logp, old_mu, old_sigma, advantages, returns, target_values, *, clip, c_surr,
-                 c_value, c_bound, c_entropy, clipped_value=True):
+                 c_value, c_bound, c_entropy, clipped_value=True, defer_finish=False):
     mu_c, std_c, val_c = _f32c(mu.detach()), _f32c(std.detach()), _f32c(value.detach())
     fixed = [_f32c(x) for x in (actions, old_logp, old_mu, old_sigma, advantages, returns, target_values)]
     B = mu_c.shape[0]
@@ -46,6 +60,10 @@
     out = torch.empty(8, dtype=torch.float32, device=mu_c.device)
     nscratch = int(API.lib.qa_ppo_loss_scratch_bytes(B))
     scratch = torch.empty(nscratch, dtype=torch.uint8, device=mu_c.device)
+    if defer_finish:
+        API.launch("ppo_loss_partials", _ptr(mu_c), _ptr(std_c), _ptr(val_c), *[_ptr(x) for x in fixed], B, 12, float(clip), float(c_surr),
+                   float(c_value), float(c_bound), float(c_entropy), int(bool(clipped_value)), _ptr(dmu), _ptr(dvalue), _ptr(scratch), nscratch, on=mu_c)
+        return out, dmu, dstd, dvalue, PpoPending(scratch, B, (float(c_surr), float(c_value), float(c_bound), float(c_entropy)), out, dstd)
     API.launch("ppo_loss", _ptr(mu_c), _ptr(std_c), _ptr(val_c), *[_ptr(x) for x in fixed], B, 12, float(clip), float(c_surr),
                float(c_value), float(c_bound), float(c_entropy), int(bool(clipped_value)),
                _ptr(dmu), _ptr(dstd), _ptr(dvalue), _ptr(out), _ptr(scratch), nscratch, on=mu_c)
@@ -289,6 +307,55 @@
         return gx, gw, gb
 
 
+class _Head1Linear(torch.autograd.Function):
+
+    @staticmethod
+    def forward(ctx, x, weight, bias):
+        xr = _rows16(x)
+        rows, k = xr.shape
+        y = torch.empty(rows, 1, dtype=torch.float32, device=x.device)
+        API.launch("head1_forward", _ptr(xr), xr.stride(0), _ptr(weight), _ptr(bias), _ptr(y), rows, k, on=x)
+        ctx.save_for_backward(xr, weight, bias)
+        return y
+
+    @staticmethod
+    def backward(ctx, gy):
+        xr, weight, bias = ctx.saved_tensors
+        _gradient_arriving(weight, bias)
+        gy = _f32c(gy)
+        rows, k = xr.shape
+        nb = (rows + 63) // 64
+        gx = torch.empty(rows, k, dtype=torch.float32, device=xr.device)
+        parts = torch.empty(nb * (k + 1), dtype=torch.float32, device=xr.device)
+        assert parts.numel() * 4 == API.lib.qa_head1_backward_scratch_bytes(rows, k)
+        defer = ctx.needs_input_grad[1] and ctx.needs_input_grad[2] and _defer_ok(weight) and _defer_ok(bias)
+        gw = gb = None
+        if not defer:
+            gw = torch.empty_like(weight, memory_format=torch.contiguous_format)
+            gb = torch.empty(1, dtype=torch.float32, device=xr.device)
+        API.launch("head1_backward", _ptr(gy), _ptr(xr), xr.stride(0), _ptr(weight), _ptr(gx), rows, k, _ptr(gw) if gw is not None else None,
+                   _ptr(gb) if gb is not None else None, _ptr(parts), parts.numel() * 4, on=xr)
+        if defer:
+            gw = _register_parts(weight, parts, nb, k + 1)
+            gb = _register_parts(bias, parts[k:], nb, k + 1)
+        return (gx if ctx.needs_input_grad[0] else None), (gw if ctx.needs_input_grad[1] else None), (gb if ctx.needs_input_grad[2] else None)
+
+
+def _rows16(t):
+    t = _rows2d(t)
+    if t.data_ptr() % 16 or t.stride(0) % 4:
+        t = t.contiguous()
+    return t
+
+
+def head1_ok(m, x):
+    return (ENABLED and HEAD1 and isinstance(m, torch.nn.Linear) and m.out_features == 1 and m.bias is not None and m.in_features % 4 == 0
+            and x.is_cuda and torch.is_grad_enabled() and x.dim() == 2 and x.dtype == torch.float32 and x.shape[1] == m.in_features
+            and m.weight.dtype == torch.float32 and m.weight.is_contiguous() and m.weight.data_ptr() % 16 == 0 and m.weight.requires_grad)
+
+
+TOP_DX_FIRST = os.environ.get("QA_TOP_DX_FIRST", "1") != "0"
+HEAD1 = os.environ.get("QA_HEAD1", "1") != "0"
 NARROW_MAX_OUT = 32
 NARROW_MIN_ROWS = 1
 
@@ -297,6 +364,8 @@
     if (ENABLED and OWN_GEMM and x.is_cuda and torch.is_grad_enabled() and x.dim() == 2 and x.dtype == torch.float32 and m.bias is not None
             and m.out_features > NARROW_MAX_OUT and m.weight.requires_grad):
         return _MlpChain.apply(x, ((ACT_NONE, 0.0),), m.weight, m.bias)
+    if head1_ok(m, x):
+        return _Head1Linear.apply(x, m.weight, m.bias)
     return narrow_linear(m, x)
 
 
@@ -490,12 +559,20 @@
         for i in range(L - 1, -1, -1):
             w = params[2 * i]
             need_w, need_b = ctx.needs_input_grad[2 + 2 * i], ctx.needs_input_grad[3 + 2 * i]
+            g_next = None
+            if i == L - 1 and TOP_DX_FIRST:
+                if i > 0:
+                    g_next = linear_backward_input_raw(g, w, acts[i], spec[i - 1][0], spec[i - 1][1])
+                elif ctx.needs_input_grad[0]:
+                    gx = linear_backward_input_raw(g, w0p if kpad else w, None, ACT_NONE)
             if need_w or need_b:
                 gw, gb = linear_backward_weight_raw(g, acts[i])
                 if i == 0 and kpad:
                     gw = gw[:, :w.shape[1]].contiguous()
                 grads[2 * i], grads[2 * i + 1] = (gw if need_w else None), (gb if need_b else None)
-            if i > 0:
+            if i == L - 1 and TOP_DX_FIRST:
+                g = g_next if i > 0 else g
+            elif i > 0:
                 g = linear_backward_input_raw(g, w, acts[i], spec[i - 1][0], spec[i - 1][1])
             elif ctx.needs_input_grad[0]:
                 gx = linear_backward_input_raw(g, w0p if kpad else w, None, ACT_NONE)
@@ -552,12 +629,16 @@
                 x = m(x)
         return x
     every = any(a in NEW_ACTS for _, a, _ in spec)
+    head1 = lambda e: HEAD1 and not every and e[1] == ACT_NONE and e[0].out_features == 1 and e[0].in_features % 4 == 0
     i = 0
     while i < len(spec):
         m, act, alpha = spec[i]
-        if every or own_layer(m.in_features, m.out_features):
+        if head1(spec[i]) and head1_ok(m, x):
+            x = _Head1Linear.apply(x, m.weight, m.bias)
+            i += 1
+        elif every or own_layer(m.in_features, m.out_features):
             j = i
-            while j < len(spec) and (every or own_layer(spec[j][0].in_features, spec[j][0].out_features)):
+            while j < len(spec) and (every or own_layer(spec[j][0].in_features, spec[j][0].out_features)) and not (j > i and head1(spec[j])):
                 j += 1
             params = []
             for mm, _, _ in spec[i:j]:
@@ -757,10 +838,15 @@
     return outs
 
 
+def scalars_ok(acc, scalars):
+    n = len(scalars)
+    return bool(ENABLED and acc.is_cuda and acc.dtype == torch.float32 and acc.is_contiguous() and acc.numel() >= n and 0 < n <= 16
+                and all(torch.is_tensor(x) and x.dtype == torch.float32 and x.numel() == 1 and x.device == acc.device for x in scalars))
+
+
 def accumulate_scalars(acc, scalars):
     n = len(scalars)
-    if not (ENABLED and acc.is_cuda and acc.dtype == torch.float32 and acc.is_contiguous() and acc.numel() >= n and n <= 16
-            and all(torch.is_tensor(x) and x.dtype == torch.float32 and x.numel() == 1 and x.device == acc.device for x in scalars)):
+    if not scalars_ok(acc, scalars):
         acc[:n].add_(torch.stack([x.reshape(()) for x in scalars]))
         return
     API.launch("accumulate_scalars", _ptr(acc), (C.c_void_p * n)(*[x.data_ptr() for x in scalars]), n, on=acc)
@@ -924,7 +1010,10 @@
     def warm(self):
         return self.step(dry=True)
 
-    def step(self, kl=None, desired_kl=0.0, factor=1.5, lr_min=1e-5, lr_max=1e-2, dry=False):
+    def ready(self):
+        return self._tab is not None
+
+    def step(self, kl=None, desired_kl=0.0, factor=1.5, lr_min=1e-5, lr_max=1e-2, dry=False, pending=None, scalars=None):
         a, b = self.first, self.second
         self.why_not = None
         if not (ENABLED and a.max_norm > 0 and b.max_norm > 0):
@@ -967,13 +1056,24 @@
         pair = _capi.QaAdamPair(ta["n"], ta["num_chunks"], pb["lr_dev"].data_ptr(), b.max_norm, kl.data_ptr() if kl is not None else None,
                                 float(desired_kl) if kl is not None else 0.0, float(factor), float(lr_min), float(lr_max))
         params = pa["params"] + pb["params"]
+        riders = ()
+        if pending is not None or scalars is not None:
+            pend_s = pending.struct() if pending is not None else None
+            sc_s = None
+            if scalars is not None:
+                acc, vals = scalars
+                sc_s = _capi.QaStepScalars(acc.data_ptr(), (C.c_void_p * _capi.ACC_MAX)(*[x.data_ptr() for x in vals]), len(vals))
+            riders = (C.byref(pend_s) if pend_s is not None else None, C.byref(sc_s) if sc_s is not None else None)
         try:
-            API.launch("clip_adam_pair_step", _ptr(m["params"]), (C.c_void_p * n)(*ptrs), _ptr(m["exp_avg"]), _ptr(m["exp_avg_sq"]), _ptr(m["steps"]), m["n"],
+            API.launch("clip_adam_pair_step_pending" if riders else "clip_adam_pair_step", _ptr(m["params"]), (C.c_void_p * n)(*ptrs), _ptr(m["exp_avg"]),
+                       _ptr(m["exp_avg_sq"]), _ptr(m["steps"]), m["n"],
                        _ptr(m["chunk_tensor"]), _ptr(m["chunk_start"]), _ptr(m["chunk_len"]), m["num_chunks"], _ptr(m["wd"]),
                        _ptr(pa["lr_dev"]), float(ta["betas"][0]), float(ta["betas"][1]), float(ta["eps"]), a.max_norm,
-                       _ptr(m["scratch"]), m["scratch"].numel(), src, stride, parts, C.byref(pair), on=params[0])
+                       _ptr(m["scratch"]), m["scratch"].numel(), src, stride, parts, C.byref(pair), *riders, on=params[0])
         finally:
             _take_pending(params)
+        if pending is not None:
+            pending.done = True
         return True
 
 
diff --git a/quadrupedal_agility_amd/rsl_rl/algorithms/gail.py b/quadrupedal_agility_amd/rsl_rl/algorithms/gail.py
--- a/quadrupedal_agility_amd/rsl_rl/algorithms/gail.py
+++ b/quadrupedal_agility_amd/rsl_rl/algorithms/gail.py
@@ -300,9 +300,9 @@
                 self._gather_srcs = flat + [self._hist_latent_all]
                 self._perm_bufs = [torch.empty(nmb * mb, x.shape[1] if x.dim() == 2 else 1, device=dev) for x in self._gather_srcs]
 
-                def front(i):
+                def front(i, apply_follows=False):
                     obs, act, val, adv, ret, logp, mu, sig, hl = (b[i * mb:(i + 1) * mb] for b in self._perm_bufs)
-                    return self._ac_forward_backward((obs, obs, act, val, adv, ret, logp, mu, sig, (None, None), None, hl))
+                    return self._ac_forward_backward((obs, obs, act, val, adv, ret, logp, mu, sig, (None, None), None, hl), apply_follows=apply_follows)
 
                 torch.cuda.synchronize()
                 for o in (self.optim_ac, self.optim_estimator):
@@ -314,9 +314,9 @@
                     epoch_graph = sync is None and self._train_chain_rows(mb) is not None and os.environ.get("QA_STEP_UNROLL", "1") != "0"
 
                     def slot(i):
-                        stats, kl = front(i)
-                        self._ac_apply(kl)
-                        fused_mod.accumulate_scalars(self._acc_ac, stats)
+                        stats, kl = front(i, apply_follows=True)
+                        if not self._ac_apply(kl, scalars=(self._acc_ac, stats)):
+                            fused_mod.accumulate_scalars(self._acc_ac, stats)
 
                     def epoch():
                         for i in range(nmb):
@@ -445,13 +445,14 @@
         if self.grad_sync is not None:
             self.grad_sync(params)
 
-    def _ac_forward_backward(self, sample):
+    def _ac_forward_backward(self, sample, apply_follows=False):
         (obs, critic_obs, actions, target_values, advantages, returns, old_logp, old_mu, old_sigma, _hid, _masks) = sample[:11]
         hist_latent = sample[11] if len(sample) > 11 else None
         ac = self.actor_critic
         fused = self._on_gpu and self.use_fused_loss
         if fused and not ac.fixed_std:
-            return self._ac_forward_backward_direct(obs, critic_obs, actions, target_values, advantages, returns, old_logp, old_mu, old_sigma, hist_latent)
+            return self._ac_forward_backward_direct(obs, critic_obs, actions, target_values, advantages, returns, old_logp, old_mu, old_sigma, hist_latent,
+                                                    apply_follows=apply_follows)
         if fused:
             mu = ac._actor_mean(obs.detach(), False)
             value = ac.evaluate(critic_obs.detach())
@@ -515,7 +516,7 @@
         return (surrogate_loss.detach(), value_loss.detach(), b_mean.detach(), ent_mean.detach(),
                 priv_reg_loss.detach(), estimator_loss.detach()), kl_mean
 
-    def _ac_forward_backward_direct(self, obs, critic_obs, actions, target_values, advantages, returns, old_logp, old_mu, old_sigma, hist_latent):
+    def _ac_forward_backward_direct(self, obs, critic_obs, actions, target_values, advantages, returns, old_logp, old_mu, old_sigma, hist_latent, apply_follows=False):
         ac = self.actor_critic
         a = self.num_prop; b = a + self.num_explicit; c = b + self.num_latent; d = c + self.num_hist * self.num_prop
         priv_reg_coef = self._priv_coef_dev if self._recording_ac else self._priv_reg_coef_now()
@@ -549,10 +550,15 @@
         mu = ac._actor_mean(obs.detach(), False)
         if self.branch_streams:
             cur.wait_stream(s_critic)
-        out, dmu, dstd, dvalue = fused_mod.ppo_loss_raw(mu, ac.std, value, actions, old_logp, old_mu, old_sigma, advantages, returns, target_values,
-                                                        clip=self.clip_param, c_surr=self.surrogate_loss_coef, c_value=self.value_loss_coef,
-                                                        c_bound=self.bounds_loss_coef, c_entropy=self.entropy_coef,
-                                                        clipped_value=self.use_clipped_value_loss)
+        defer = bool(apply_follows and self.grad_sync is None and self._step_pair is not None and self.use_fused_loss and self._step_pair.ready()
+                     and os.environ.get("QA_DEFER_PPO_FINISH", "1") != "0")
+        self._ppo_pending = None
+        out, dmu, dstd, dvalue, *pending = fused_mod.ppo_loss_raw(mu, ac.std, value, actions, old_logp, old_mu, old_sigma, advantages, returns, target_values,
+                                                                  clip=self.clip_param, c_surr=self.surrogate_loss_coef, c_value=self.value_loss_coef,
+                                                                  c_bound=self.bounds_loss_coef, c_entropy=self.entropy_coef,
+                                                                  clipped_value=self.use_clipped_value_loss, defer_finish=defer)
+        if pending:
+            self._ppo_pending = pending[0]
         if self.branch_streams:
             cur.wait_stream(s_small)
             if not self._recording_ac:
@@ -620,17 +626,22 @@
         adaptive = self.desired_kl is not None and self.schedule == "adaptive"
         return (out[1], out[2], out[3], out[4], priv_reg_loss, estimator_loss), (out[5] if adaptive else None)
 
-    def _ac_apply(self, kl_mean):
+    def _ac_apply(self, kl_mean, scalars=None):
         sides = getattr(self, "_chain_sides", None)
+        pending, self._ppo_pending = getattr(self, "_ppo_pending", None), None
+        if scalars is not None and not fused_mod.scalars_ok(*scalars):
+            scalars = None
         if sides is not None:
             with sides.fork(0):
                 self._step_estimator.step()
         elif (self._step_pair is not None and self.use_fused_loss and (kl_mean is None or (kl_mean.dtype == torch.float32 and kl_mean.is_contiguous()))
-              and self._step_pair.step(kl_mean, self.desired_kl)):
+              and self._step_pair.step(kl_mean, self.desired_kl, pending=pending, scalars=scalars)):
             if fused_mod.pending_grads():
                 fused_mod.flush_pending_grads()
-            return
-        else:
+            return scalars is not None
+        else:
+            if pending is not None:
+                pending.finish()
             self._step_estimator.step()
         if kl_mean is not None:
             self._apply_kl_schedule(kl_mean)
@@ -639,9 +650,10 @@
             sides.join()
         if fused_mod.pending_grads():
             fused_mod.flush_pending_grads()
+        return False
 
     def update_actor_critic(self, sample):
-        stats, kl_mean = self._ac_forward_backward(sample)
+        stats, kl_mean = self._ac_forward_backward(sample, apply_follows=self.grad_sync is None)
         if self.grad_sync is not None:
             params = list(self.estimator.parameters()) + list(self.actor_critic.parameters())
             synced = self.grad_sync(params, extra=[kl_mean] if kl_mean is not None else None)
```
